# biodatageeks/datafusion-bio-functions

Measured on AMD Instinct MI355X. Metric: overlap-pairs/sec + probe-rows/sec, IntervalJoinExec 100Mx1M, higher is better.
Workload: dtype int32; 1 GPU; join_100Mx1M_24contigs; probe_rows_per_gpu=100000000, build_rows_per_gpu=1000000, contigs=24, pairs_per_gpu=37210484, parallelism=partition-per-gpu x1, gather=False, build_overlap=True

## Files before the change

datafusion-bio-functions_amd/csrc/ivx_capi.hip:

```cpp
#include "ivx_internal.hpp"
#include <cstdlib>
#include <atomic>
#include <chrono>
#include <cstring>
#include <mutex>
#include <new>
#include <thread>
#include <condition_variable>
#include <deque>


void ivx_ctx::join_tail()
{
    if (!tail_pending) return;
    (void)hipStreamWaitEvent(stream, tail_ev, 0);
    tail_pending = false;
}

ivx_status ivx_ctx::get_scratch(int slot, size_t bytes, void **out)
{
    if (tail_pending && slot != WS_SORTHIST && slot != WS_T0 && slot != WS_T1 && slot != WS_T2) join_tail();
    ivx_buf &b = scratch[slot];
    if (sub_plan.valid && ((sub_plan.slots >> slot) & 1)) sub_plan.valid = false;
    if (join_plan.valid && ((join_plan.rows.slots >> slot) & 1)) join_plan.valid = false;
    if (bytes < 256) bytes = 256;
    if (b.cap < bytes) {
        size_t want = bytes + bytes / 8;
        if (mem_limit) {
            const u64 others = reserved() - b.cap;
            if (others + bytes > mem_limit)
                return fail(IVX_ERR_OOM, "Resources exhausted: failed to reserve " + std::to_string(bytes) + " bytes of device scratch (" +
                                         std::to_string(others) + " bytes reserved, limit " + std::to_string(mem_limit) + ")");
            if (others + want > mem_limit) want = bytes;
        }
        if (b.p) { (void)hipStreamSynchronize(stream); if (aux) (void)hipStreamSynchronize(aux); (void)hipFree(b.p); b.p = nullptr; scratch_bytes -= b.cap; b.cap = 0; }
        hipError_t e = hipMalloc(&b.p, want);
        if (e != hipSuccess) { want = bytes; e = hipMalloc(&b.p, want); }
        if (e != hipSuccess) { b.p = nullptr; return fail_hip("hipMalloc(scratch)", e); }
        b.cap = want; scratch_bytes += want;
    }
    *out = b.p;
    return IVX_OK;
}

ivx_status ivx_ctx::get_pinned(int slot, size_t bytes, void **out)
{
    ivx_buf &b = pinned[slot];
    if (bytes < 256) bytes = 256;
    if (b.cap < bytes) {
        if (b.p) { (void)hipStreamSynchronize(stream); (void)hipHostFree(b.p); b.p = nullptr; b.cap = 0; }
        hipError_t e = hipHostMalloc(&b.p, bytes, hipHostMallocDefault);
        if (e != hipSuccess) { b.p = nullptr; return fail_hip("hipHostMalloc", e); }
        b.cap = bytes;
    }
    *out = b.p;
    return IVX_OK;
}

namespace {
struct PoolBuf { void *p; size_t cap; int device; };
std::mutex g_pool_mu;
std::vector<PoolBuf> g_pool;
constexpr size_t POOL_MAX_BUFS = 96;

void *pool_take(int device, size_t bytes, size_t *cap)
{
    std::lock_guard<std::mutex> lk(g_pool_mu);
    size_t best = g_pool.size();
    for (size_t i = 0; i < g_pool.size(); i++) {
        const PoolBuf &b = g_pool[i];
        if (b.device != device || b.cap < bytes || b.cap > 2 * bytes + 4096) continue;
        if (best == g_pool.size() || b.cap < g_pool[best].cap) best = i;
    }
    if (best == g_pool.size()) return nullptr;
    void *p = g_pool[best].p;
    *cap = g_pool[best].cap;
    g_pool.erase(g_pool.begin() + best);
    return p;
}

void pool_give(int device, void *p, size_t cap)
{
    void *drop = nullptr;
    {
        std::lock_guard<std::mutex> lk(g_pool_mu);
        g_pool.push_back({p, cap, device});
        if (g_pool.size() > POOL_MAX_BUFS) { drop = g_pool.front().p; g_pool.erase(g_pool.begin()); }
    }
    if (drop) (void)hipFree(drop);
}

void pool_drop(int device)
{
    std::vector<void *> drop;
    {
        std::lock_guard<std::mutex> lk(g_pool_mu);
        for (size_t i = 0; i < g_pool.size();)
            if (g_pool[i].device == device) { drop.push_back(g_pool[i].p); g_pool.erase(g_pool.begin() + i); }
            else i++;
    }
    for (void *p : drop) (void)hipFree(p);
}
}

ivx_status ivx_index_alloc(ivx_ctx *ctx, ivx_index *ix, size_t bytes, void **out)
{
    if (bytes < 256) bytes = 256;
    if (ctx->mem_limit && ctx->reserved() + bytes > ctx->mem_limit)
        return ctx->fail(IVX_ERR_OOM, "Resources exhausted: failed to reserve " + std::to_string(bytes) + " bytes for the index (" +
// ... 125 lines not shown
    c->stream = c->own_stream;
    if (const char *e = getenv("IVX_BUILD_OVERLAP")) c->overlap = e[0] == '1';
    *out = c;
    return IVX_OK;
}

extern "C" void ivx_ctx_free(ivx_ctx *c)
{
    if (!c) return;
    (void)hipSetDevice(c->device);
    (void)hipStreamSynchronize(c->stream);
    if (c->aux) (void)hipStreamSynchronize(c->aux);
    for (auto &b : c->scratch) if (b.p) (void)hipFree(b.p);
    for (auto &b : c->pinned) if (b.p) (void)hipHostFree(b.p);
    if (c->d_scalars) (void)hipFree(c->d_scalars);
    if (c->h_scalars) (void)hipHostFree(c->h_scalars);
    if (c->ev0) (void)hipEventDestroy(c->ev0);
    if (c->ev1) (void)hipEventDestroy(c->ev1);
    if (c->own_stream) (void)hipStreamDestroy(c->own_stream);
    if (c->aux) (void)hipStreamDestroy(c->aux);
    if (c->ev_fork) (void)hipEventDestroy(c->ev_fork);
    if (c->tail_ev) (void)hipEventDestroy(c->tail_ev);
    delete c;
}

extern "C" const char *ivx_last_error(const ivx_ctx *c) { return c ? c->err.c_str() : "null ctx"; }

extern "C" ivx_status ivx_ctx_set_stream(ivx_ctx *c, void *hip_stream)
{
    if (!c) return IVX_ERR_INVALID;
    if (c->tail_pending) { (void)hipStreamSynchronize(c->aux); c->tail_pending = false; }
    c->stream = (hipStream_t)hip_stream;
    return IVX_OK;
}

extern "C" ivx_status ivx_ctx_use_own_stream(ivx_ctx *c)
{
    if (!c) return IVX_ERR_INVALID;
    if (c->tail_pending) { (void)hipStreamSynchronize(c->aux); c->tail_pending = false; }
    c->stream = c->own_stream;
    return IVX_OK;
}

extern "C" ivx_status ivx_ctx_set_build_overlap(ivx_ctx *c, int on)
{
    if (!c) return IVX_ERR_INVALID;
    c->overlap = on != 0;
    return IVX_OK;
}

extern "C" ivx_status ivx_ctx_synchronize(ivx_ctx *c)
{
    if (!c) return IVX_ERR_INVALID;
    if (c->tail_pending) { IVX_HIP(c, hipStreamSynchronize(c->aux)); c->tail_pending = false; }
    IVX_HIP(c, hipStreamSynchronize(c->stream));
    return IVX_OK;
}

extern "C" ivx_status ivx_ctx_metrics(const ivx_ctx *c, ivx_metrics *out)
{
    if (!c || !out) return IVX_ERR_INVALID;
    *out = c->metrics;
    return IVX_OK;
}

extern "C" void ivx_ctx_reset_metrics(ivx_ctx *c) { if (c) c->metrics = ivx_metrics{}; }

extern "C" ivx_status ivx_ctx_set_memory_limit(ivx_ctx *c, uint64_t bytes)
{
    if (!c) return IVX_ERR_INVALID;
    c->mem_limit = bytes;
    return IVX_OK;
}

extern "C" uint64_t ivx_ctx_reserved_bytes(const ivx_ctx *c) { return c ? c->reserved() : 0; }

extern "C" ivx_status ivx_ctx_trim(ivx_ctx *c, uint64_t keep_bytes)
{
    if (!c) return IVX_ERR_INVALID;
    IVX_HIP(c, hipSetDevice(c->device));
    IVX_HIP(c, hipStreamSynchronize(c->stream));
    if (c->aux) { IVX_HIP(c, hipStreamSynchronize(c->aux)); c->tail_pending = false; }
    c->sub_plan.valid = false; c->join_plan.valid = false;
    while (c->scratch_bytes > keep_bytes) {
        int big = -1;
        for (int i = 0; i < IVX_NSCRATCH; i++)
            if (c->scratch[i].p && (big < 0 || c->scratch[i].cap > c->scratch[big].cap)) big = i;
        if (big < 0) break;
        IVX_HIP(c, hipFree(c->scratch[big].p));
        c->scratch_bytes -= c->scratch[big].cap;
        c->scratch[big] = ivx_buf{};
    }
    pool_drop(c->device);
    return IVX_OK;
}

extern "C" double ivx_ctx_last_kernel_ms(const ivx_ctx *cc)
{
    ivx_ctx *c = const_cast<ivx_ctx *>(cc);
    if (!c) return -1.0;
    if (c->last_ms < 0.0) {
        float ms = 0.f;
        if (hipEventSynchronize(c->ev1) == hipSuccess && hipEventElapsedTime(&ms, c->ev0, c->ev1) == hipSuccess) c->last_ms = ms;
    }
    return c->last_ms;
}


ivx_status ivx_count_build(ivx_ctx *ctx, ivx_index *ix, const u32 *key, const i32 *s, const i32 *e, u64 n);
ivx_status ivx_coverage_build(ivx_ctx *ctx, ivx_index *ix, const u32 *key, const i32 *s, const i32 *e, u64 n);
ivx_status ivx_nearest_build(ivx_ctx *ctx, ivx_index *ix, const u32 *key, const i32 *s, const i32 *e, u64 n);

extern "C" ivx_status ivx_index_build(ivx_ctx *ctx, int kind, int mem, const uint32_t *key, const int32_t *start,
                                      const int32_t *end, uint64_t n, uint32_t n_keys, ivx_index **out)
{
    if (!ctx) return IVX_ERR_INVALID;
    if (!out) return ctx->fail(IVX_ERR_INVALID, "null out");
    *out = nullptr;
    if (kind < IVX_KIND_OVERLAP || kind > IVX_KIND_NEAREST) return ctx->fail(IVX_ERR_INVALID, "bad index kind");
    if (mem != IVX_MEM_HOST && mem != IVX_MEM_DEVICE) return ctx->fail(IVX_ERR_INVALID, "bad mem");
    if (n && (!start || !end)) return ctx->fail(IVX_ERR_INVALID, "null coordinate column");
    if (n > 0xFFFFFFFEull) return ctx->fail(IVX_ERR_INVALID, "build side exceeds UInt32 index capacity");
    if (n_keys == 0) n_keys = 1;
    if (!key) n_keys = 1;
    if (kind == IVX_KIND_NEAREST && n >= 0x80000000ull) return ctx->fail(IVX_ERR_INVALID, "nearest index: more than 2^31-1 rows");
    IVX_HIP(ctx, hipSetDevice(ctx->device));
    ivx_index *ix = new (std::nothrow) ivx_index();
    static std::atomic<u64> next_serial{1};
    if (ix) ix->serial = next_serial.fetch_add(1);
    if (!ix) return ctx->fail(IVX_ERR_OOM, "host allocation failed");
    ix->kind = kind; ix->device = ctx->device; ix->n = n; ix->nkeys = n_keys;
    CallMetrics cm(ctx, true, n);
    ctx->building_bytes = 0;
    const u32 *dk; const i32 *ds, *de;
    ivx_status st = stage_in(ctx, mem, WS_IN_KEY, key, n, &dk);
    if (st == IVX_OK) st = stage_in(ctx, mem, WS_IN_START, start, n, &ds);
    if (st == IVX_OK) st = stage_in(ctx, mem, WS_IN_END, end, n, &de);
    if (st == IVX_OK) {
        KernelTimer t(ctx);
        switch (kind) {
        case IVX_KIND_OVERLAP: st = ivx_join_build(ctx, ix, dk, ds, de, n, mem == IVX_MEM_DEVICE); break;
        case IVX_KIND_COUNT: st = ivx_count_build(ctx, ix, dk, ds, de, n); break;
        case IVX_KIND_COVERAGE: st = ivx_coverage_build(ctx, ix, dk, ds, de, n); break;
        default: st = ivx_nearest_build(ctx, ix, dk, ds, de, n); break;
        }
    }
    if (st == IVX_OK && hipStreamSynchronize(ctx->stream) != hipSuccess) st = ctx->fail(IVX_ERR_HIP, "index build failed on device");
    ctx->building_bytes = 0;
    if (st != IVX_OK) { ivx_index_free(ix); return st; }
    ix->owner_bytes = ctx->live_index_bytes;
    ix->owner_bytes->fetch_add(ix->bytes, std::memory_order_relaxed);
    ctx->metrics.build_mem_used += ix->bytes;
    *out = ix;
    return IVX_OK;
}

extern "C" void ivx_index_free(ivx_index *ix)
{
    if (!ix) return;
    if (ix->ready) { (void)hipEventSynchronize(ix->ready); (void)hipEventDestroy(ix->ready); }
    for (size_t i = 0; i < ix->allocs.size(); i++) pool_give(ix->device, ix->allocs[i], ix->alloc_caps[i]);
    if (ix->owner_bytes) ix->owner_bytes->fetch_sub(ix->bytes, std::memory_order_relaxed);
    delete ix;
}

extern "C" uint64_t ivx_index_rows(const ivx_index *ix) { return ix ? ix->n : 0; }
extern "C" uint64_t ivx_index_device_bytes(const ivx_index *ix) { return ix ? ix->bytes : 0; }

extern "C" ivx_status ivx_index_layout(ivx_ctx *ctx, const ivx_index *ix, uint32_t *out, uint32_t n_out)
{
    if (!ctx) return IVX_ERR_INVALID;
    if (!ix) return ctx->fail(IVX_ERR_INVALID, "null index");
    if (n_out && !out) return ctx->fail(IVX_ERR_INVALID, "null out");
    if (ix->device != ctx->device) return ctx->fail(IVX_ERR_INVALID, "index lives on another device");
    u32 w[IVX_LAYOUT_WORDS] = {};
    w[IVX_LAYOUT_KIND] = (u32)ix->kind;
    if (ix->kind != IVX_KIND_NEAREST && ix->jv.hdr != nullptr) {
        IVX_HIP(ctx, hipSetDevice(ctx->device));
        if (ix->ready != nullptr) IVX_HIP(ctx, hipStreamWaitEvent(ctx->stream, ix->ready, 0));
        u32 h[HDR_WORDS];
        IVX_HIP(ctx, hipMemcpyAsync(h, ix->jv.hdr, sizeof(h), hipMemcpyDeviceToHost, ctx->stream));
        IVX_HIP(ctx, hipStreamSynchronize(ctx->stream));
        const u32 nlev = h[HDR_NLEV] < IVX_MAXL ? h[HDR_NLEV] : IVX_MAXL;
        u32 levrows = 0;
        for (u32 l = 0; l < nlev; l++) if (h[HDR_LEVCNT + l]) levrows |= 1u << l;
        w[IVX_LAYOUT_SH0] = h[HDR_SH0];
        w[IVX_LAYOUT_NLEV] = h[HDR_NLEV];
        w[IVX_LAYOUT_LEVROWS] = levrows;
        w[IVX_LAYOUT_RCELLS] = h[HDR_NREG] ? h[HDR_RCELLS] : 0u;
        w[IVX_LAYOUT_RCS] = h[HDR_NREG] ? h[HDR_CS] : 0xFFFFFFFFu;
        w[IVX_LAYOUT_NREG] = h[HDR_NREG];
        w[IVX_LAYOUT_PK24] = h[HDR_PK24];
        w[IVX_LAYOUT_SLOW] = h[HDR_SLOW];
        w[IVX_LAYOUT_FG] = h[HDR_FG];
        w[IVX_LAYOUT_FBITS] = h[HDR_FG] != 0xFFFFFFFFu ? h[HDR_FBITS] : 0u;
        w[IVX_LAYOUT_NROUTE_NREG] = ix->nroute_nreg;
        w[IVX_LAYOUT_LBUILD] = h[HDR_LBUILD];
    }
    for (u32 i = 0; i < n_out && i < (u32)IVX_LAYOUT_WORDS; i++) out[i] = w[i];
    return IVX_OK;
}


static bool rowval_routed_ok(u64 n)
{
    if (const char *f = getenv("IVX_JOIN_PATH")) return !strcmp(f, "routed");
    return n >= (1u << 21);
}

static ivx_status overlap_common(ivx_ctx *ctx, const ivx_index *ix, int mem, int mode,
                                 const u32 *key, const i32 *start, const i32 *end, u64 n,
                                 u32 *per_row, u8 *exists, u32 *bidx, u32 *pidx, u64 cap, u64 *total)
{
    IVX_TRY(check_probe_args(ctx, ix, IVX_KIND_OVERLAP, mem, start, end, n, true));
    CallMetrics cm(ctx, false, n);
    const u32 *dk = nullptr; const i32 *ds = nullptr, *de = nullptr;
    bool regions = ix->jv_nreg > 0 && (mode == JP_COUNT || mode == JP_FILL) && n >= (1u << 21);
    bool rowval = ix->jv_nreg > 0 && ix->jv_nreg <= IVX_MAXREG_WIDE && (mode == JP_PER_ROW || mode == JP_EXISTS) && n >= (1u << 21);
    if (const char *f = getenv("IVX_JOIN_PATH")) {
        if (!strcmp(f, "direct")) regions = rowval = false;
        else if (!strcmp(f, "regions")) {
            regions = ix->jv_nreg > 0 && (mode == JP_COUNT || mode == JP_FILL);
            rowval = ix->jv_nreg > 0 && ix->jv_nreg <= IVX_MAXREG_WIDE && (mode == JP_PER_ROW || mode == JP_EXISTS);
        }
    }
    const void *in[3] = {key, start, end};
    ivx_join_plan &pl = ctx->join_plan;
    const bool planned = regions && mode == JP_FILL && pl.valid && !getenv("IVX_NO_PLAN") && pl.mem == mem && memcmp(pl.in, in, sizeof(in)) == 0 && pl.n == n &&
                         pl.ix == (const void *)ix && pl.ix_serial == ix->serial && pl.stream == ctx->stream;
    if (ix->ready != nullptr && !(regions && !planned)) IVX_HIP(ctx, hipStreamWaitEvent(ctx->stream, ix->ready, 0));
    if (!planned) {
        IVX_TRY(stage_in(ctx, mem, WS_IN_KEY, key, n, &dk));
        IVX_TRY(stage_in(ctx, mem, WS_IN_START, start, n, &ds));
        IVX_TRY(stage_in(ctx, mem, WS_IN_END, end, n, &de));
    }
    u32 *d_row = nullptr, *d_b = nullptr, *d_p = nullptr; u8 *d_ex = nullptr;
    IVX_TRY(stage_out(ctx, mem, WS_OUT_A, per_row, n, &d_row));
    IVX_TRY(stage_out(ctx, mem, WS_OUT_B, exists, n, &d_ex));
    IVX_TRY(stage_out(ctx, mem, WS_OUT_C, bidx, cap, &d_b));
    IVX_TRY(stage_out(ctx, mem, WS_OUT_D, pidx, cap, &d_p));
    const bool defer_clear = regions && !planned;
    if (!defer_clear) IVX_HIP(ctx, hipMemsetAsync(ctx->d_scalars, 0, 2 * sizeof(u64), ctx->stream));
    {
        KernelTimer t(ctx);
        if (regions) {
            if (!planned) pl.valid = false;
            const ivx_status st = ivx_join_probe_regions(ctx, ix->jv, ix->jv_nreg, mode, dk, ds, de, n, d_b, d_p, cap, ctx->d_scalars, planned, ix->jv_filter, ix->jv_pk24,
                                                         ix->jv_fast_unknown ? 2 : (ix->jv_fast ? 1 : 0), planned ? nullptr : ix->ready, defer_clear);
            if (st != IVX_OK) { pl.valid = false; return st; }
            if (mode == JP_COUNT && pl.valid) { memcpy(pl.in, in, sizeof(in)); pl.mem = mem; pl.n = n; pl.ix = ix; pl.ix_serial = ix->serial; pl.stream = ctx->stream; }
        }
        else if (rowval) IVX_TRY(ivx_rowval_probe_regions(ctx, ix->jv, ix->jv_nreg, mode == JP_PER_ROW ? IVX_RV_PER_ROW : IVX_RV_EXISTS, dk, ds, de, n, 0,
                                                          mode == JP_PER_ROW ? (void *)d_row : (void *)d_ex, ctx->d_scalars, ix->jv_filter, ix->jv_pk24, ix->jv_fast && !ix->jv_fast_unknown));
        else if (n && (mode == JP_PER_ROW || mode == JP_EXISTS) && ix->nroute_nreg > 0 && rowval_routed_ok(n))
            IVX_TRY(ivx_join_rowval_routed(ctx, ix, mode, dk, ds, de, n, d_row, d_ex, ctx->d_scalars));
        else IVX_TRY(ivx_join_probe(ctx, ix->jv, mode, dk, ds, de, n, d_row, d_ex, d_b, d_p, cap, ctx->d_scalars));
    }
    u64 tot = 0;
    if (mode != JP_EXISTS) {
        IVX_HIP(ctx, hipMemcpyAsync(ctx->h_scalars, ctx->d_scalars, 2 * sizeof(u64), hipMemcpyDeviceToHost, ctx->stream));
        IVX_HIP(ctx, hipStreamSynchronize(ctx->stream));
        tot = ctx->h_scalars[0];
        if (ctx->h_scalars[1]) { ctx->join_plan.valid = false; return ctx->fail(IVX_ERR_HIP, "internal error: the probe met an unpublished page of routed rows"); }
    }
    if (mode == JP_COUNT && regions && pl.valid) pl.total = tot;
    if (total) *total = tot;
    if (mode == JP_FILL && tot > cap) return ctx->fail(IVX_ERR_CAPACITY, "pair buffers too small");
    cm.out(mode == JP_FILL ? tot : (mode == JP_COUNT ? 0 : n));
    if (planned) pl.valid = false;
    IVX_TRY(copy_out(ctx, mem, per_row, d_row, n));
    IVX_TRY(copy_out(ctx, mem, exists, d_ex, n));
    if (mode == JP_FILL) { IVX_TRY(copy_out(ctx, mem, bidx, d_b, tot)); IVX_TRY(copy_out(ctx, mem, pidx, d_p, tot)); }
    if (mem == IVX_MEM_HOST) IVX_HIP(ctx, hipStreamSynchronize(ctx->stream));
    return IVX_OK;
}

extern "C" ivx_status ivx_probe_overlap_count(ivx_ctx *ctx, const ivx_index *ix, int mem, const uint32_t *key,
                                              const int32_t *start, const int32_t *end, uint64_t n,
                                              uint32_t *per_row, uint64_t *total)
{
    return overlap_common(ctx, ix, mem, per_row ? JP_PER_ROW : JP_COUNT, key, start, end, n, per_row, nullptr, nullptr, nullptr, 0, total);
}

__global__ void k_add_base(u32 *__restrict__ p, u64 n, u32 base)
{
    for (u64 i = (u64)blockIdx.x * blockDim.x + threadIdx.x; i < n; i += (u64)gridDim.x * blockDim.x) p[i] += base;
}

struct HostCopier {
    struct Job { void *dst; const void *src; size_t bytes; hipEvent_t ev; };
    std::mutex mu; std::condition_variable cv, cv_done; std::deque<Job> jobs; bool closed = false; hipError_t herr = hipSuccess;
    u64 done = 0;
    hipStream_t cs = nullptr; std::thread th; std::vector<hipEvent_t> evs; bool started = false;
    hipError_t start(int device)
    {
        const hipError_t e = hipStreamCreateWithFlags(&cs, hipStreamNonBlocking);
        if (e != hipSuccess) return e;
        try {
        th = std::thread([this, device]() {
            (void)hipSetDevice(device);
            for (;;) {
                Job j;
                { std::unique_lock<std::mutex> lk(mu); cv.wait(lk, [&] { return closed || !jobs.empty(); }); if (jobs.empty()) return; j = jobs.front(); jobs.pop_front(); }
                hipError_t e2 = j.ev ? hipStreamWaitEvent(cs, j.ev, 0) : hipSuccess;
                if (e2 == hipSuccess && j.bytes) e2 = hipMemcpyAsync(j.dst, j.src, j.bytes, hipMemcpyDeviceToHost, cs);
                if (e2 == hipSuccess) e2 = hipStreamSynchronize(cs);
                { std::lock_guard<std::mutex> lk(mu); if (e2 != hipSuccess) herr = e2; done++; }
                cv_done.notify_all();
            }
        });
        } catch (...) { (void)hipStreamDestroy(cs); cs = nullptr; return hipErrorOutOfMemory; }
        started = true;
        return hipSuccess;
    }
    hipError_t mark(hipStream_t st, hipEvent_t *ev)
    {
        hipError_t e = hipEventCreateWithFlags(ev, hipEventDisableTiming);
        if (e != hipSuccess) return e;
        evs.push_back(*ev);
        return hipEventRecord(*ev, st);
    }
    void push(void *dst, const void *src, size_t bytes, hipEvent_t ev)
    {
        { std::lock_guard<std::mutex> lk(mu); jobs.push_back(Job{dst, src, bytes, ev}); }
        cv.notify_all();
    }
    void wait_until(u64 k) { std::unique_lock<std::mutex> lk(mu); cv_done.wait(lk, [&] { return done >= k; }); }
    hipError_t finish()
    {
        if (!started) return hipSuccess;
        { std::lock_guard<std::mutex> lk(mu); closed = true; }
        cv.notify_all();
        th.join();
        for (hipEvent_t e : evs) (void)hipEventDestroy(e);
        (void)hipStreamDestroy(cs);
        started = false;
        return herr;
    }
    ~HostCopier() { (void)finish(); }
};

static ivx_status overlap_fill_host_chunked(ivx_ctx *ctx, const ivx_index *ix, const u32 *key, const i32 *start, const i32 *end, u64 n,
                                            u32 *bidx, u32 *pidx, u64 cap, u64 *written, u32 nchunk)
{
    IVX_TRY(check_probe_args(ctx, ix, IVX_KIND_OVERLAP, IVX_MEM_HOST, start, end, n));
    hipStream_t st = ctx->stream;
// ... 724 lines not shown
```

datafusion-bio-functions_amd/csrc/ivx_internal.hpp:

```cpp
#pragma once
#include <hip/hip_runtime.h>
#include <stdint.h>
#include <atomic>
#include <memory>
#include <string>
#include <vector>
#include "../../include/ivx.h"

typedef uint8_t u8;
typedef uint32_t u32;
typedef int32_t i32;
typedef uint64_t u64;
typedef int64_t i64;

#define IVX_WAVE 64

struct ivx_buf { void *p = nullptr; size_t cap = 0; };

enum { IVX_NSCRATCH = 56, IVX_NPIN = 4 };

struct ivx_sub_plan {
    bool valid = false;
    u64 slots = 0;
    int mem = 0;
    const void *in[6] = {};
    u64 nl = 0, nr = 0, nh = 0, total = 0;
    u32 nkeys = 0;
    int strict = 0;
    hipStream_t stream = nullptr;
    const u32 *lk, *lrow, *rk, *hk, *hj;
    const i64 *lsv, *lev, *rsv, *hrs, *hpm;
    const void *sm;
    const u64 *offs;
    const u32 *plan_hlo; const i64 *plan_tail;
};

struct PageTab { u32 *ptab; u32 pstride, lgpg; };
struct ivx_route_ctl {
    u32 rcur[1024];
    u32 pool_next, pad0[3];
    u32 rest_n[2], pad1[2];
    u32 rfirst[1032];
    u32 cfirst[1032];
};
struct FpRest;
enum {
    IVX_ROWS_FLAT = 0,
    IVX_ROWS_PAGED,
    IVX_ROWS_TABLE
};
struct ivx_routed {
    int form = IVX_ROWS_FLAT;
    const u64 *se = nullptr;
    const u32 *ids = nullptr;
    const unsigned short *cidx = nullptr;
    const u32 *rfirst = nullptr;
    u32 nblk = 1, chunk = 0, ndig = 0;
    const u32 *unsorted = nullptr;
    PageTab pt{nullptr, 0u, 0u};
    bool packed = false;
    u32 rowbits = 32;
    bool all_routed = false;
    ivx_route_ctl *ctl = nullptr;
    FpRest *rest = nullptr; u64 *rest_rows = nullptr;
    const uint2 *vtab = nullptr;
    const i32 *ds = nullptr, *de = nullptr;
    u32 adj = 0;
    u64 slots = 0;
};

struct ivx_join_plan {
    bool valid = false;
    int mem = 0;
    const void *in[3] = {};
    u64 n = 0;
    u64 total = 0;
    const void *ix = nullptr; u64 ix_serial = 0;
    hipStream_t stream = nullptr;
    ivx_routed rows;
};

struct ivx_ctx {
    int device = 0;
    hipStream_t own_stream = nullptr;
    hipStream_t stream = nullptr;
    hipEvent_t ev0 = nullptr, ev1 = nullptr;
    double last_ms = 0.0;
    std::string err;
    ivx_buf scratch[IVX_NSCRATCH];
    ivx_buf pinned[IVX_NPIN];
    u64 *d_scalars = nullptr;
    u64 *h_scalars = nullptr;
    ivx_sub_plan sub_plan;
    ivx_join_plan join_plan;
    ivx_metrics metrics{};
    u64 mem_limit = 0;
    u64 fill_hint = 0;
    u64 scratch_bytes = 0, building_bytes = 0;
    hipStream_t aux = nullptr;
    hipEvent_t ev_fork = nullptr, tail_ev = nullptr;
    bool overlap = false, tail_pending = false;
    void join_tail();
    std::shared_ptr<std::atomic<u64>> live_index_bytes = std::make_shared<std::atomic<u64>>(0);
    u64 reserved() const { return scratch_bytes + building_bytes + live_index_bytes->load(std::memory_order_relaxed); }

    ivx_status fail(ivx_status st, const std::string &msg) { err = msg; return st; }
    ivx_status fail_hip(const char *what, hipError_t e)
    {
        err = std::string(what) + ": " + hipGetErrorString(e);
        return e == hipErrorOutOfMemory ? IVX_ERR_OOM : IVX_ERR_HIP;
    }
    ivx_status get_scratch(int slot, size_t bytes, void **out);
    ivx_status get_pinned(int slot, size_t bytes, void **out);
};

#define IVX_HIP(ctx, call)                                              \
    do {                                                                \
        hipError_t e__ = (call);                                        \
        if (e__ != hipSuccess) return (ctx)->fail_hip(#call, e__);      \
    } while (0)

#define IVX_TRY(call)                                                   \
    do {                                                                \
        ivx_status s__ = (call);                                        \
        if (s__ != IVX_OK) return s__;                                  \
    } while (0)

enum {
    WS_IN_KEY = 0, WS_IN_START, WS_IN_END, WS_IN2_KEY, WS_IN2_START, WS_IN2_END,
    WS_OUT_A, WS_OUT_B, WS_OUT_C, WS_OUT_D, WS_OUT_E, WS_OUT_F, WS_OUT_G, WS_OUT_H,
    WS_SCAN0, WS_SCAN1, WS_SCAN2,
    WS_GRID0, WS_GRID1, WS_GRID2,
    WS_SORTHIST,
    WS_SA0, WS_SA1, WS_SA2, WS_SB0, WS_SB1, WS_SB2,
    WS_RA0, WS_RA1, WS_RA2, WS_RB0, WS_RB1, WS_RB2,
    WS_T0, WS_T1, WS_T2, WS_T3, WS_T4, WS_T5, WS_T6, WS_T7, WS_T8, WS_T9,
    WS_IN3_KEY, WS_IN3_START, WS_IN3_END, WS_IN3_WEIGHT, WS_IN_KEYLEN
};
static_assert(WS_IN_KEYLEN < IVX_NSCRATCH, "scratch slot ids must fit the context's slot array");

#ifndef IVX_LSTEP
#define IVX_LSTEP 2
#endif
#define IVX_MAXL (32 / IVX_LSTEP)
#define IVX_SH_MIN 4

struct ivx_ent { i32 s, e; u32 row; };

enum { HDR_SH0 = 0, HDR_NLEV = 1, HDR_NBINS = 2, HDR_CS = 3 , HDR_NREG = 4,
       HDR_RCELLS = 5 , HDR_RMUL_LO = 6, HDR_RMUL_HI = 7 , HDR_LEVCNT = 8 ,
       HDR_FG = 8 + IVX_MAXL , HDR_FBITS = 9 + IVX_MAXL ,
       HDR_PK24 = 10 + IVX_MAXL ,
       HDR_SLOW = 11 + IVX_MAXL ,
       HDR_LBUILD = 12 + IVX_MAXL ,
       HDR_BADKEY = 13 + IVX_MAXL ,
       HDR_WORDS = 14 + IVX_MAXL };
#define IVX_FBITS_MAX (1u << 24)
#define IVX_MAXREG 255
#define IVX_MAXREG_WIDE 1023
#define IVX_MAXREG2 65025u
#define IVX_REG_CS_MAX 13

#ifndef IVX_RP_ECAP
#define IVX_RP_ECAP 6144
#endif
#define IVX_RP_HALO 8u
struct ivx_regdesc { u32 k; i32 origin; u32 span, lb, slo, shi, e0, ne; i32 rbase;  };

struct JoinIndexView {
    const i32 *origin;
    const u32 *span;
    const u32 *kcnt;
    const u32 *lbase;
    const u32 *binstart;
    const ivx_ent *ent;
    const u32 *hdr;
    const u32 *kreg;
    const u32 *rkey;
    const ivx_regdesc *rdesc;
    const u32 *fbits;
    const u32 *fbase;
    u32 nkeys;
};

struct RankGridView {
    const i32 *origin;
    const u32 *span;
    const u32 *kcnt;
    const u32 *koff;
    const u32 *kbase;
    const u32 *binstart;
    const i32 *val;
    const u32 *hdr;
    u32 nkeys;
};

struct CoverageView {
    RankGridView first, last;
    const i64 *pw;
    const i32 *nfirst, *nlast;
};

struct ivx_nrec { i32 a, b; u32 row; i32 pmax; };

struct NearestView {
    RankGridView by_start, by_end, pmax;
    const ivx_nrec *rs;
    const ivx_nrec *re;
    JoinIndexView ov;
};

struct ivx_index {
    u64 serial = 0;
    int kind = 0;
    int device = 0;
    u64 n = 0;
    u32 nkeys = 0;
    size_t bytes = 0;
    std::shared_ptr<std::atomic<u64>> owner_bytes;
    std::vector<void *> allocs;
    std::vector<size_t> alloc_caps;
    JoinIndexView jv{};
    u32 jv_nreg = 0;
    bool jv_filter = false;
    bool jv_pk24 = false;
    bool jv_fast = false;
    bool jv_fast_unknown = false;
    hipEvent_t ready = nullptr;
    RankGridView gs{}, ge{};
    CoverageView cv{};
    NearestView nv{};
    JoinIndexView nroute{};
    u32 nroute_nreg = 0;
    int flags = 0;
};
enum { IVX_IXF_REGION_ROWVAL = 1 };

ivx_status ivx_scan_exclusive_u32(ivx_ctx *ctx, u32 *data, u64 n, const u32 *skip = nullptr);
ivx_status ivx_scan_exclusive_u64(ivx_ctx *ctx, u64 *data, u64 n);

ivx_status ivx_join_build(ivx_ctx *ctx, ivx_index *ix, const u32 *key, const i32 *s, const i32 *e, u64 n, bool overlap = false);
ivx_status ivx_join_probe(ivx_ctx *ctx, const JoinIndexView &jv, int mode,
                          const u32 *key, const i32 *s, const i32 *e, u64 n,
                          u32 *per_row, u8 *exists, u32 *ob, u32 *op, u64 cap, u64 *d_cursor);
enum { JP_COUNT = 0, JP_PER_ROW = 1, JP_EXISTS = 2, JP_FILL = 3 };
ivx_status ivx_join_probe_regions(ivx_ctx *ctx, const JoinIndexView &jv, u32 nreg, int mode,
                                  const u32 *key, const i32 *s, const i32 *e, u64 n,
                                  u32 *ob, u32 *op, u64 cap, u64 *d_cursor, bool planned = false, bool has_filter = false, bool pk24 = false,
                                  int fast = 0 , hipEvent_t ready = nullptr,
                                  bool clear_cursor = false );

enum { IVX_RV_COUNT = 0, IVX_RV_COVERAGE = 1, IVX_RV_PER_ROW = 2, IVX_RV_EXISTS = 3 };
ivx_status ivx_route_view_build(ivx_ctx *ctx, ivx_index *ix, const i32 *origin, const u32 *span, const u32 *kcnt);
void ivx_route_view_ready(ivx_ctx *ctx, ivx_index *ix);
ivx_status ivx_join_rowval_routed(ivx_ctx *ctx, const ivx_index *ix, int mode, const u32 *key, const i32 *s, const i32 *e, u64 n,
                                  u32 *per_row, u8 *exists, u64 *d_total);
ivx_status ivx_unroute_u32(ivx_ctx *ctx, const ivx_routed &r, u64 n, const u32 *vb, u32 *out32, u8 *out8);
ivx_status ivx_route_rows(ivx_ctx *ctx, const JoinIndexView &rv, const u32 *key, const i32 *s, const i32 *e, u64 n, u32 adj, ivx_routed *out);
ivx_status ivx_unroute_pair(ivx_ctx *ctx, const ivx_routed &r, u64 n, const u32 *vb, const i64 *vd, u32 *ob, u32 *op, i64 *od, i64 dflt);
ivx_status ivx_rowval_probe_regions(ivx_ctx *ctx, const JoinIndexView &jv, u32 nreg, int kind,
                                    const u32 *key, const i32 *s, const i32 *e, u64 n, int strict, void *out, u64 *d_total,
                                    bool has_filter = false, bool pk24 = false, bool fast = false);

ivx_status ivx_mark_probe(ivx_ctx *ctx, const JoinIndexView &jv, const u32 *key, const i32 *s, const i32 *e, u64 n, u32 *marks);
ivx_status ivx_mark_probe_regions(ivx_ctx *ctx, const JoinIndexView &jv, u32 nreg, const u32 *key, const i32 *s, const i32 *e, u64 n,
                                  u32 *marks, bool has_filter, bool pk24, bool fast, bool *took);
ivx_status ivx_bits_mark_device(ivx_ctx *ctx, const u32 *idx, u64 n, u32 *bits, u64 n_bits);
ivx_status ivx_bits_select_device(ivx_ctx *ctx, const u32 *bits, u64 n_bits, int want_set, u32 *out, u64 cap, u64 *n_out);

ivx_status ivx_depth_device(ivx_ctx *ctx, const u32 *rkey, const u32 *rpos, const u32 *rflags, const u32 *rmapq,
                            const i32 *cigar_offsets, const u32 *cigar_ops, u64 n_reads,
                            const u32 *skey, const u32 *sstart, const u32 *send, const i32 *sweight, u64 n_seg,
                            u32 nkeys, const u32 *key_len, u32 filter_flag, u32 min_mapq,
                            u32 *ok, u32 *os, u32 *oe, i32 *oc, u64 cap, u64 *n_out);

ivx_status ivx_index_alloc(ivx_ctx *ctx, ivx_index *ix, size_t bytes, void **out);
```

datafusion-bio-functions_amd/csrc/ivx_join.hip:

```cpp
#include <cstdlib>
#include <cstring>
#include "ivx_device.hpp"
#include "ivx_grid.hpp"
#include "ivx_join.hpp"

namespace {

constexpr int BT = 256;

constexpr int LB_T = 1024;
constexpr int LB_ROWS = 4;
constexpr u32 LB_TILE = LB_T * LB_ROWS;
constexpr u32 LB_STRIDE = IVX_MAXREG_WIDE + 1;
constexpr u32 LB_CCAP = 8192;
constexpr u32 LB_MAXTILES = 1024;
constexpr int LB_KEEP = (IVX_RP_ECAP + LB_T - 1) / LB_T;
constexpr u64 LB_MIN_ROWS = 1u << 14, LB_MAX_ROWS = (u64)LB_MAXTILES * LB_TILE;
static_assert(LB_STRIDE == LB_T && LB_TILE <= 4096 && LB_CCAP == (1u << IVX_REG_CS_MAX), "k_lbuild_tiles: one table word per thread, 12-bit ranks");
static inline u32 lb_tstride(u32 ntiles) { return ntiles | 1u; }


__device__ __forceinline__ u32 cells_of(u32 cnt, u32 span, u32 sh) { return cnt ? (sh >= 32 ? 1u : (span >> sh) + 1u) : 0u; }

__global__ __launch_bounds__(1024) void k_join_layout(const i32 *kmin, const i32 *kmax, const u32 *kcnt, u32 nkeys, u64 n,
// ... 542 lines not shown


ivx_status ivx_route_view_build(ivx_ctx *ctx, ivx_index *ix, const i32 *origin, const u32 *span, const u32 *kcnt)
{
    hipStream_t st = ctx->stream;
    const u32 nkeys = ix->nkeys;
    u32 *kreg, *rkey, *rhdr;
    IVX_TRY(ivx_index_alloc(ctx, ix, ((size_t)nkeys + 1) * sizeof(u32), (void **)&kreg));
    IVX_TRY(ivx_index_alloc(ctx, ix, ((size_t)IVX_MAXREG_WIDE + 1) * sizeof(u32), (void **)&rkey));
    IVX_TRY(ivx_index_alloc(ctx, ix, HDR_WORDS * sizeof(u32), (void **)&rhdr));
    IVX_HIP(ctx, hipMemsetAsync(rhdr, 0, HDR_WORDS * sizeof(u32), st));
    hipLaunchKernelGGL(k_nroute_layout, dim3(1), dim3(1024), 0, st, origin, span, kcnt, nkeys, kreg, rkey, rhdr);
    IVX_HIP(ctx, hipMemcpyAsync(ctx->h_scalars + 48, rhdr, HDR_WORDS * sizeof(u32), hipMemcpyDeviceToHost, st));
    ix->nroute = JoinIndexView{};
    ix->nroute.origin = origin; ix->nroute.span = span; ix->nroute.kcnt = kcnt; ix->nroute.kreg = kreg; ix->nroute.rkey = rkey;
    ix->nroute.hdr = rhdr; ix->nroute.nkeys = nkeys;
    IVX_HIP(ctx, hipGetLastError());
    return IVX_OK;
}
void ivx_route_view_ready(ivx_ctx *ctx, ivx_index *ix) { ix->nroute_nreg = ((const u32 *)(ctx->h_scalars + 48))[HDR_NREG]; }

ivx_status ivx_join_rowval_routed(ivx_ctx *ctx, const ivx_index *ix, int mode, const u32 *key, const i32 *s, const i32 *e, u64 n,
                                  u32 *per_row, u8 *exists, u64 *d_total)
{
    hipStream_t st = ctx->stream;
    ivx_routed R;
    IVX_TRY(ivx_route_rows(ctx, ix->nroute, key, s, e, n, 0u, &R));
    u32 *vb;
    IVX_TRY(ctx->get_scratch(WS_T2, n * sizeof(u32), (void **)&vb));
    const u32 grid = (ivx_stream_grid(n, PT * 4, 1280u) + 7u) & ~7u;
    hipLaunchKernelGGL(k_overlap_rowval_routed, dim3(grid), dim3(PT), 0, st, ix->jv, ix->nroute.rkey, ix->nroute_nreg, R.se, R.rfirst, R.nblk,
                       mode == JP_EXISTS ? 1 : 0, vb, (unsigned long long *)d_total, R.unsorted);
    IVX_TRY(ivx_unroute_u32(ctx, R, n, vb, per_row, exists));
    const u32 g2 = ivx_stream_grid(n, PTILE, 256 * 8);
    if (mode == JP_PER_ROW) hipLaunchKernelGGL((k_probe_overlap<JP_PER_ROW, PI>), dim3(g2), dim3(PT), 0, st, ix->jv, key, s, e, n, per_row, exists, (u32 *)nullptr, (u32 *)nullptr, (u64)0, (unsigned long long *)d_total, R.unsorted);
    else hipLaunchKernelGGL((k_probe_overlap<JP_EXISTS, PI>), dim3(g2), dim3(PT), 0, st, ix->jv, key, s, e, n, per_row, exists, (u32 *)nullptr, (u32 *)nullptr, (u64)0, (unsigned long long *)d_total, R.unsorted);
    IVX_HIP(ctx, hipGetLastError());
    return IVX_OK;
}

ivx_status ivx_join_build(ivx_ctx *ctx, ivx_index *ix, const u32 *key, const i32 *s, const i32 *e, u64 n, bool overlap)
{
    const u32 nkeys = ix->nkeys;
    hipStream_t st = ctx->stream;
    const u64 maxcells = 2 * n + (IVX_LSTEP >= 4 ? n / 4 : n) + (u64)IVX_MAXL * nkeys + 64;
    if (maxcells + 1 >= 0xFFFFFFFFull) return ctx->fail(IVX_ERR_INVALID, "build side too large for 32-bit cell ids");

    i32 *origin; u32 *span, *kcnt, *lbase, *binstart, *hdr, *kreg, *rkey, *fbase, *fbits; ivx_ent *ent; ivx_regdesc *rdesc;
    IVX_TRY(ivx_index_alloc(ctx, ix, nkeys * sizeof(i32), (void **)&origin));
    IVX_TRY(ivx_index_alloc(ctx, ix, nkeys * sizeof(u32), (void **)&span));
    IVX_TRY(ivx_index_alloc(ctx, ix, nkeys * sizeof(u32), (void **)&kcnt));
    IVX_TRY(ivx_index_alloc(ctx, ix, (size_t)IVX_MAXL * nkeys * sizeof(u32), (void **)&lbase));
    IVX_TRY(ivx_index_alloc(ctx, ix, (maxcells + 1) * sizeof(u32), (void **)&binstart));
    IVX_TRY(ivx_index_alloc(ctx, ix, HDR_WORDS * sizeof(u32), (void **)&hdr));
    IVX_TRY(ivx_index_alloc(ctx, ix, ((size_t)nkeys + 1) * sizeof(u32), (void **)&kreg));
    size_t regcap = (size_t)(n / (IVX_RP_ECAP / 2)) + (size_t)(maxcells >> IVX_REG_CS_MAX) + 2 * (size_t)nkeys + 64;
    regcap = regcap <= IVX_MAXREG + 1 ? (size_t)IVX_MAXREG + 1 : (regcap > (size_t)IVX_MAXREG2 + 1 ? (size_t)IVX_MAXREG2 + 1 : regcap);
    IVX_TRY(ivx_index_alloc(ctx, ix, regcap * sizeof(u32), (void **)&rkey));
    IVX_TRY(ivx_index_alloc(ctx, ix, regcap * sizeof(ivx_regdesc), (void **)&rdesc));
    IVX_TRY(ivx_index_alloc(ctx, ix, (n ? n : 1) * sizeof(ivx_ent), (void **)&ent));
    const size_t fwords = IVX_FBITS_MAX / 32 + 4;
    IVX_TRY(ivx_index_alloc(ctx, ix, nkeys * sizeof(u32), (void **)&fbase));
    IVX_TRY(ivx_index_alloc(ctx, ix, fwords * sizeof(u32), (void **)&fbits));

    i32 *kmin, *kmax; u32 *cellid, *rank, *errflag;
    IVX_TRY(ctx->get_scratch(WS_GRID0, nkeys * sizeof(i32), (void **)&kmin));
    IVX_TRY(ctx->get_scratch(WS_GRID1, nkeys * sizeof(i32), (void **)&kmax));
    const char *benv = getenv("IVX_BUILD");
    const bool lb_try = n >= LB_MIN_ROWS && n <= LB_MAX_ROWS && !(benv && !strcmp(benv, "global"));
    const u32 lb_tiles = lb_try ? (u32)((n + LB_TILE - 1) / LB_TILE) : 0u;
    IVX_TRY(ctx->get_scratch(WS_GRID2, (n ? n : 1) * (lb_try ? sizeof(ivx_ent) : sizeof(u32)), (void **)&cellid));
    const size_t tabbytes = (size_t)lb_tstride(lb_tiles) * LB_STRIDE * sizeof(u32);
    IVX_TRY(ctx->get_scratch(WS_T9, (n ? n : 1) * sizeof(u32) > tabbytes ? (n ? n : 1) * sizeof(u32) : tabbytes, (void **)&rank));
    errflag = (u32 *)(ctx->d_scalars + 8);
    u32 *lenhist = (u32 *)(ctx->d_scalars + 32);

    ivx_zero_ranges zr{{errflag, lenhist, hdr}, {1u, 34u, (u32)HDR_WORDS}};
    const char *fenv = getenv("IVX_FILTER");
    const int filter_mode = !fenv ? 1 : !strcmp(fenv, "0") ? 0 : !strcmp(fenv, "force") ? 2 : 1;
    static_assert((IVX_FBITS_MAX / 32 + 4) % 4 == 0, "the bitmap is cleared in 16-byte words");
    if (filter_mode) { zr.big = (uint4 *)fbits; zr.nbig = (u32)(fwords / 4); }
    IVX_TRY(ivx_keystats_len(ctx, key, s, n, nkeys, kmin, kmax, kcnt, errflag, 1u, e, lenhist, &zr));
    const u32 grid = ivx_stream_grid(n, BT * 2, 16384);
    hipLaunchKernelGGL(k_join_layout, dim3(1), dim3(1024), 0, st, kmin, kmax, kcnt, nkeys, n, origin, span, lbase, hdr, maxcells, kreg, rkey, (const u32 *)lenhist, (u32)(regcap - 1), fbase, filter_mode, lb_try ? 1 : 0, (const u32 *)errflag);
    if (filter_mode) hipLaunchKernelGGL(k_join_filter, dim3(grid), dim3(BT), 0, st, key, s, e, n, nkeys, (const i32 *)origin, (const u32 *)span, (const u32 *)fbase, (const u32 *)hdr, fbits);
    const bool want_route = ix->kind == IVX_KIND_OVERLAP && n >= (4u << 20);
    overlap = overlap && ctx->overlap && ctx->aux != nullptr && !want_route && n >= (1u << 16);
    hipStream_t tail_st = st;
    struct TailGuard {
        ivx_ctx *c; bool armed = false;
        ~TailGuard() { if (armed) (void)hipStreamSynchronize(c->aux); }
    } guard{ctx};
    bool q_lds = lb_try, q_global = true;
    if (overlap) {
        ctx->join_tail();
        IVX_HIP(ctx, hipEventRecord(ctx->ev_fork, st));
        IVX_HIP(ctx, hipStreamWaitEvent(ctx->aux, ctx->ev_fork, 0));
        tail_st = ctx->aux;
        IVX_HIP(ctx, hipMemcpyAsync(ctx->h_scalars + 32, hdr, HDR_WORDS * sizeof(u32), hipMemcpyDeviceToHost, st));
        IVX_HIP(ctx, hipStreamSynchronize(st));
        if (((const u32 *)(ctx->h_scalars + 32))[HDR_BADKEY]) return ctx->fail(IVX_ERR_INVALID, "build key id >= n_keys");
        q_lds = lb_try && ((const u32 *)(ctx->h_scalars + 32))[HDR_LBUILD] != 0;
        q_global = !q_lds;
        guard.armed = true;
    }
    if (q_lds)
        hipLaunchKernelGGL(k_lbuild_tiles, dim3(lb_tiles), dim3(LB_T), 0, tail_st, key, s, e, n, nkeys, (const i32 *)origin, (const u32 *)kreg, hdr,
                           (ivx_ent *)cellid, rank, lb_tstride(lb_tiles), binstart, maxcells + 1);
    else
        IVX_HIP(ctx, hipMemsetAsync(binstart, 0, (maxcells + 1) * sizeof(u32), tail_st));
    if (q_global) {
        hipLaunchKernelGGL(k_join_count, dim3(grid), dim3(BT), 0, tail_st, key, s, e, n, nkeys, origin, lbase, hdr, binstart, cellid, rank);
        const hipStream_t keep = ctx->stream;
        ctx->stream = tail_st;
        const ivx_status sst = ivx_scan_exclusive_u32(ctx, binstart, maxcells + 1, hdr + HDR_LBUILD);
        ctx->stream = keep;
        IVX_TRY(sst);
        hipLaunchKernelGGL(k_join_scatter, dim3(grid), dim3(BT), 0, tail_st, s, e, n, (const u32 *)binstart, (const u32 *)cellid, (const u32 *)rank, ent, (const u32 *)hdr);
    }
    if (q_lds) {
        const u32 rgrid = regcap - 1 < IVX_MAXREG_WIDE ? (u32)(regcap - 1) : (u32)IVX_MAXREG_WIDE;
        hipLaunchKernelGGL(k_lbuild_regions, dim3(rgrid), dim3(LB_T), 0, tail_st, (const i32 *)origin, (const u32 *)span, (const u32 *)lbase, (const u32 *)kreg,
                           (const u32 *)rkey, (const u32 *)hdr, nkeys, (const ivx_ent *)cellid, (const u32 *)rank, lb_tiles, lb_tstride(lb_tiles), binstart, ent);
    }
    hipLaunchKernelGGL(k_join_regdesc, dim3((u32)((regcap + 255) / 256)), dim3(256), 0, tail_st, origin, span, lbase, hdr, kreg, rkey, binstart, rdesc);
    IVX_HIP(ctx, hipGetLastError());
    if (overlap) {
        if (ix->ready == nullptr) IVX_HIP(ctx, hipEventCreateWithFlags(&ix->ready, hipEventDisableTiming));
        IVX_HIP(ctx, hipEventRecord(ix->ready, ctx->aux));
        IVX_HIP(ctx, hipEventRecord(ctx->tail_ev, ctx->aux));
        ctx->tail_pending = true;
        ix->jv_fast_unknown = true;
    }
    if (want_route) IVX_TRY(ivx_route_view_build(ctx, ix, origin, span, kcnt));

    if (!overlap) {
        IVX_HIP(ctx, hipMemcpyAsync(ctx->h_scalars + 32, hdr, HDR_WORDS * sizeof(u32), hipMemcpyDeviceToHost, st));
        IVX_HIP(ctx, hipStreamSynchronize(st));
    }
    if (((const u32 *)(ctx->h_scalars + 32))[HDR_BADKEY]) return ctx->fail(IVX_ERR_INVALID, "build key id >= n_keys");
    ix->jv_nreg = ((const u32 *)(ctx->h_scalars + 32))[HDR_NREG];
    ix->jv_filter = ((const u32 *)(ctx->h_scalars + 32))[HDR_FG] != 0xFFFFFFFFu;
    ix->jv_pk24 = ((const u32 *)(ctx->h_scalars + 32))[HDR_PK24] != 0;
    ix->jv_fast = ((const u32 *)(ctx->h_scalars + 32))[HDR_SLOW] == 0 && ix->jv_nreg > 0;
    if (want_route) ivx_route_view_ready(ctx, ix);
    guard.armed = false;

    ix->jv.origin = origin; ix->jv.span = span; ix->jv.kcnt = kcnt; ix->jv.lbase = lbase;
    ix->jv.binstart = binstart; ix->jv.ent = ent; ix->jv.hdr = hdr; ix->jv.nkeys = nkeys;
    ix->jv.kreg = kreg; ix->jv.rkey = rkey; ix->jv.rdesc = rdesc;
    ix->jv.fbits = fbits; ix->jv.fbase = fbase;
    return IVX_OK;
}

ivx_status ivx_join_probe(ivx_ctx *ctx, const JoinIndexView &jv, int mode,
                          const u32 *key, const i32 *s, const i32 *e, u64 n,
                          u32 *per_row, u8 *exists, u32 *ob, u32 *op, u64 cap, u64 *d_cursor)
{
    if (n == 0) return IVX_OK;
    unsigned long long *cur = (unsigned long long *)d_cursor;
    const bool small = n <= (1u << 18);
    const u32 grid = small ? (u32)((n + PT - 1) / PT) : ivx_stream_grid(n, PTILE, 256 * 8);
#define IVX_PROBE_LAUNCH(M_) do { \
        if (small) hipLaunchKernelGGL((k_probe_overlap<M_, 1>), dim3(grid), dim3(PT), 0, ctx->stream, jv, key, s, e, n, per_row, exists, ob, op, cap, cur, (const u32 *)nullptr); \
        else hipLaunchKernelGGL((k_probe_overlap<M_, PI>), dim3(grid), dim3(PT), 0, ctx->stream, jv, key, s, e, n, per_row, exists, ob, op, cap, cur, (const u32 *)nullptr); \
    } while (0)
    switch (mode) {
    case JP_COUNT: IVX_PROBE_LAUNCH(JP_COUNT); break;
    case JP_PER_ROW: IVX_PROBE_LAUNCH(JP_PER_ROW); break;
    case JP_EXISTS: IVX_PROBE_LAUNCH(JP_EXISTS); break;
    default: IVX_PROBE_LAUNCH(JP_FILL); break;
    }
#undef IVX_PROBE_LAUNCH
    IVX_HIP(ctx, hipGetLastError());
    return IVX_OK;
}
```

datafusion-bio-functions_amd/csrc/ivx_join.hpp:

```cpp
#pragma once
#include "ivx_device.hpp"

__device__ __forceinline__ u32 level_of(i32 s, i32 e, u32 sh0, u32 nlev)
{
    i64 len = (i64)e - (i64)s;
    if (len <= 0) return 0;
    u32 bits = 64 - __clzll((u64)len);
    u32 l = bits <= sh0 ? 0 : (bits - sh0 + IVX_LSTEP - 1) / IVX_LSTEP;
    return l < nlev ? l : nlev - 1;
}

__device__ __forceinline__ u32 cell_of(const i32 *origin, const u32 *lbase, u32 nkeys, u32 k, i32 s, u32 l, u32 sh0)
{
    const u32 sh = sh0 + IVX_LSTEP * l;
    const u32 off = (u32)((i64)s - (i64)origin[k]);
    return lbase[(u64)l * nkeys + k] + (sh >= 32 ? 0u : off >> sh);
}

template <class F>
__device__ __forceinline__ void walk_ent(const JoinIndexView &ix, u32 sh0, u32 lev0, u32 nlev, u32 k, i32 qs, i32 qe, F &&f)
{
    if (k >= ix.nkeys) return;
    if (ix.kcnt[k] == 0) return;
    const i32 origin = ix.origin[k];
    const u32 span = ix.span[k];
    const i64 hi64 = (i64)qe - (i64)origin;
    if (hi64 < 0) return;
    for (u32 l = lev0; l < nlev; l++) {
        if (ix.hdr[HDR_LEVCNT + l] == 0) continue;
        const u32 sh = sh0 + IVX_LSTEP * l;
        u32 blo = 0, bhi = 0;
        if (sh < 32) {
            const u32 ncell = (span >> sh) + 1u;
            const i64 lo64 = (i64)qs - ((i64)1 << sh) + 1 - (i64)origin;
            const i64 bl = lo64 <= 0 ? 0 : (lo64 >> sh);
            const i64 bh = hi64 >> sh;
            if (bl >= (i64)ncell) continue;
            blo = (u32)bl;
            bhi = bh >= (i64)ncell ? ncell - 1u : (u32)bh;
            if (blo > bhi) continue;
        }
        const u32 base = ix.lbase[(u64)l * ix.nkeys + k];
        const u32 a = ix.binstart[base + blo], b = ix.binstart[base + bhi + 1];
        for (u32 j = a; j < b; j++) {
            const ivx_ent x = ix.ent[j];
            if (x.s <= qe && x.e >= qs) f(x);
        }
    }
}
template <class F>
__device__ __forceinline__ void walk(const JoinIndexView &ix, u32 sh0, u32 lev0, u32 nlev, u32 k, i32 qs, i32 qe, F &&f)
{
    walk_ent(ix, sh0, lev0, nlev, k, qs, qe, [&](const ivx_ent &x) { f(x.row); });
}

__device__ __forceinline__ void mark_bit(u32 *bits, u32 i)
{
    u32 *w = bits + (i >> 5);
    const u32 b = 1u << (i & 31u);
    if ((*w & b) == 0u) atomicOr(w, b);
}
```

datafusion-bio-functions_amd/csrc/ivx_regions_probe.hip:

```cpp
#include "ivx_regions.hpp"

namespace {


#ifndef IVX_RP_B
#define IVX_RP_B 8
#endif
#ifndef IVX_RP_RING
#define IVX_RP_RING 512
#endif
#ifndef IVX_RP_ECAP
#define IVX_RP_ECAP 6144
#endif
constexpr int RP_B = IVX_RP_B;
constexpr u32 RP_HALO = IVX_RP_HALO;
constexpr u32 RP_CCAP = 8192 + RP_HALO + 2;
constexpr u32 RP_ECAP = IVX_RP_ECAP;
constexpr u32 RP_RING = IVX_RP_RING;
constexpr u32 RP_NSLOT = 4;
constexpr u32 RP_NPG = 64;
constexpr u32 RP_STASH = 48;
constexpr u32 FD_SLOT_SHIFT = 13;
#ifndef IVX_FD_HEAD
#define IVX_FD_HEAD 3
// ... 221 lines not shown
                if (!(qe[q] < qs[q])) walk(q, [&](u32, bool, i32, i32) { v++; });
            } else if (KIND == RV_MATCHES) {
                walk(q, [&](u32, bool, i32, i32) { v++; });
            } else {
                const i32 a = rv_wadd(qe[q], 1), b = rv_wsub(qs[q], 1);
                walk(q, [&](u32, bool, i32 first, i32 last) {
                    const i32 d = rv_wsub(a < last ? a : last, b > first ? b : first);
                    v = (u32)rv_wadd((i32)v, d > 1 ? d : 1);
                });
            }
        }
        val[q] = v;
    }
}

__device__ __forceinline__ void round_publish(const ProbeLds &L, u32 mine, u32 round, u32 wv, unsigned long long *cursor)
{
    if (lane_id() != 0) return;
    const u32 sl = round % RP_NSLOT;
    L.s_wcnt[sl][wv] = mine;
    const u32 before = __hip_atomic_fetch_add(&L.s_arrive[sl], 1u, __ATOMIC_ACQ_REL, __HIP_MEMORY_SCOPE_WORKGROUP);
    if (before != RP_W - 1) return;
    u32 tot = 0;
#pragma unroll
    for (int w = 0; w < RP_W; w++) tot += L.s_wcnt[sl][w];
    L.s_base[sl] = tot ? atomicAdd(cursor, (unsigned long long)tot) : 0ull;
    __hip_atomic_store(&L.s_arrive[sl], 0u, __ATOMIC_RELAXED, __HIP_MEMORY_SCOPE_WORKGROUP);
    __hip_atomic_store(&L.s_ready[sl], round + 1u, __ATOMIC_RELEASE, __HIP_MEMORY_SCOPE_WORKGROUP);
}

__device__ __forceinline__ u64 round_wait(const ProbeLds &L, u32 round, u32 wv, u64 cap, bool &fits)
{
    const u32 sl = round % RP_NSLOT;
    while (__hip_atomic_load(&L.s_ready[sl], __ATOMIC_ACQUIRE, __HIP_MEMORY_SCOPE_WORKGROUP) != round + 1u)
        __builtin_amdgcn_s_sleep(1);
    const u64 base = L.s_base[sl];
    u64 g = base;
    u32 tot = 0;
#pragma unroll
    for (int w = 0; w < RP_W; w++) { const u32 c = L.s_wcnt[sl][w]; if (w < (int)wv) g += c; tot += c; }
    fits = base + tot <= cap;
    return g;
}

__device__ __forceinline__ void round_copy_out(const ProbeLds &L, u32 mine, u32 start, u32 round, u32 wv,
                                               u32 *ob, u32 *op, u64 cap)
{
    bool fits;
    const u64 g = round_wait(L, round, wv, cap, fits);
    if (!mine || !fits) return;
    for (u32 t = lane_id(); t < mine; t += IVX_WAVE) {
        const u64 x = L.s_q[wv][(start + t) & (RP_RING - 1)];
        ob[g + t] = (u32)x; op[g + t] = (u32)(x >> 32);
    }
}

#define IVX_PROBE_LDS(FILL)                                                                          \
    __shared__ unsigned short s_off[RP_CCAP];                                                        \
    __shared__ u64 s_ent[RP_ECAP];                                                                   \
    __shared__ u32 s_row[RP_ECAP];                                                                   \
    __shared__ u64 s_q[FILL ? RP_W : 1][RP_RING];                                                    \
    __shared__ u32 s_wpos[RP_W];                                                                     \
    __shared__ u32 s_wcnt[RP_NSLOT][RP_W];                                                           \
    __shared__ unsigned long long s_base[RP_NSLOT];                                                  \
    __shared__ u32 s_arrive[RP_NSLOT], s_ready[RP_NSLOT];                                            \
    if (threadIdx.x < RP_W) s_wpos[threadIdx.x] = 0;                                                 \
    if (threadIdx.x < RP_NSLOT) { s_arrive[threadIdx.x] = 0; s_ready[threadIdx.x] = 0; }             \
    ProbeLds L{s_off, s_ent, s_row, s_q, s_wpos, s_wcnt, s_base, s_arrive, s_ready};

__global__ void k_pick_rows(const u32 *__restrict__ rfirst, u32 nreg, u64 hint, u32 force, u32 *bsel)
{
    const u32 routed = rfirst[nreg];
    const float per_row = (float)((double)hint / (double)(routed ? routed : 1u));
    *bsel = force ? force : per_row <= 0.40f ? 8u : per_row <= 0.8f ? 4u : per_row <= 1.6f ? 2u : 1u;
}

template <int MODE, int B, bool IDENT, bool PAGED = false, bool PK = false>
__global__ __launch_bounds__(RP_T) void k_probe_regions(JoinIndexView ix, const void *__restrict__ rows_a, const void *__restrict__ rows_b,
                                                        const u32 *__restrict__ offs, u32 nblk, u32 vpb,
                                                        u32 *__restrict__ ob, u32 *__restrict__ op, u64 cap,
                                                        unsigned long long *cursor, u32 prow_stride, u32 adj,
                                                        const u32 *unsorted, PageTab pt = PageTab{nullptr, 0u, 0u},
                                                        const u32 *bsel = nullptr, const i32 *__restrict__ ps_in = nullptr, const i32 *__restrict__ pe_in = nullptr,
                                                        u32 rowbits = 32, const u32 *only_if_set = nullptr)
{
    constexpr bool FILL = MODE == 1;
    if (only_if_set != nullptr && *only_if_set == 0u) return;
    const u32 rowmask = rowbits >= 32 ? 0xFFFFFFFFu : (1u << rowbits) - 1u;
    const u32 maxlen = pk_maxlen(rowbits);
    static_assert(!PK || PAGED, "packed rows come from the one-pass partition");
    if (bsel != nullptr && *bsel != (u32)B) return;
    if ((unsorted != nullptr && *unsorted == 0) != IDENT) return;
    static_assert(!(IDENT && PAGED), "paged rows are never read in place");
    __shared__ u32 s_pg[RP_NPG];
    u32 pg_first = 0;
    auto row_at = [&](u64 i, u32, u64 rf) -> u64 {
        if (!PAGED) return i;
        const u32 x = (u32)(i - rf);
        const u32 pg = s_pg[(x >> pt.lgpg) - pg_first] - 1u;
        return ((u64)pg << pt.lgpg) + (x & ((1u << pt.lgpg) - 1u));
    };
    auto pages_load = [&](u64 lo, u64 &c_hi, u32 r, u64 rf) {
        if (!PAGED) return;
        __syncthreads();
        pg_first = (u32)(lo - rf) >> pt.lgpg;
        const u64 lim = (rf + ((u64)(pg_first + RP_NPG) << pt.lgpg)) & ~63ull;
        if (c_hi > lim) c_hi = lim;
        const u32 npg = ((u32)(c_hi - 1 - rf) >> pt.lgpg) - pg_first + 1u;
        if (threadIdx.x < npg) {
            u32 v = pt.ptab[(u64)r * pt.pstride + pg_first + threadIdx.x];
            if (v == 0u) { v = 1u; if (cursor != nullptr) atomicOr((unsigned int *)(cursor + 1), 1u); }
            s_pg[threadIdx.x] = v;
        }
        __syncthreads();
    };
    auto row_se = [&](u64 i) -> u64 {
        if (IDENT) return (u64)(u32)((u32)((const i32 *)rows_a)[i] + adj) | ((u64)(u32)((u32)((const i32 *)rows_b)[i] - adj) << 32);
        return ((const u64 *)rows_a)[i];
    };
    auto row_id = [&](u64 i, u64 at) -> u32 { return IDENT ? (u32)i : ((const u32 *)rows_b)[at * prow_stride]; };
    constexpr u32 WB = IVX_WAVE * B;
    IVX_PROBE_LDS(FILL)
    const u32 wv = threadIdx.x / IVX_WAVE, ln = lane_id();
    const u32 nreg = ix.hdr[HDR_NREG];
    __shared__ u32 s_rfirst[IVX_MAXREG_WIDE + 2];
    const bool rf_lds = nreg <= IVX_MAXREG_WIDE;
    if (rf_lds) for (u32 t = threadIdx.x; t <= nreg; t += RP_T) s_rfirst[t] = offs[(u64)t * nblk];
    __syncthreads();
    auto rfirst = [&](u32 r) -> u32 { return rf_lds ? s_rfirst[r] : offs[(u64)r * nblk]; };
    const u64 total_rows = rfirst(nreg);
    const u32 nvb = gridDim.x * vpb;
    u32 loaded_r = 0xFFFFFFFFu;
    Slice S;
    slice_init(ix, S, L);
    u32 round = 0;
    u32 pend_mine = 0, pend_start = 0;
    for (u32 vb = blockIdx.x * vpb; vb < (blockIdx.x + 1) * vpb; vb++) {
        u64 lo = total_rows * vb / nvb;
        const u64 hi = total_rows * (vb + 1) / nvb;
        u64 wcur = 0;
        if (lo < hi) {
            u32 r;
            {
                u32 a = 0, b = nreg;
                while (a < b) { const u32 m = (a + b + 1) >> 1; if (rfirst(m) <= lo) a = m; else b = m - 1; }
                r = a;
            }
            for (; lo < hi; r++) {
                const u64 rend = rfirst(r + 1);
                u64 c_hi = hi < rend ? hi : rend;
                if (c_hi <= lo) continue;
                u64 nx[B]; u32 nxr[B];
                u64 b0 = lo + (u64)wv * IVX_WAVE;
                const u64 rf = PAGED ? rfirst(r) : 0;
                pages_load(lo, c_hi, r, rf);
                u64 nat0 = 0, cat0 = 0;
                auto prefetch = [&](u64, u64 bl) -> bool {
                    if (PAGED) {
                        const u64 i0 = bl + ln, i7 = i0 + (u64)(B - 1) * (RP_W * IVX_WAVE);
                        const u32 x0 = (u32)(i0 - rf), x7 = (u32)(i7 - rf);
                        const bool one = i7 < c_hi && (x0 >> pt.lgpg) == (x7 >> pt.lgpg);
                        if (__ballot(!one) == 0) {
                            const u64 at0 = row_at(i0, r, rf);
                            nat0 = at0;
#pragma unroll
                            for (int q = 0; q < B; q++) {
                                const u64 at = at0 + (u64)q * (RP_W * IVX_WAVE);
                                nx[q] = row_se(at);
                                nxr[q] = (FILL && !PK) ? row_id(i0 + (u64)q * (RP_W * IVX_WAVE), at) : 0u;
                            }
// ... 125 lines not shown
    {
        const u32 c = c_lo + i / SUB, sb = i % SUB;
        while (c >= s_cfirst[r + 1]) r++;
        first = (c - s_cfirst[r]) * FP_CHUNK + wv * (8u * IVX_WAVE) + sb * WB;
        const u32 rows = rcur[r];
        cnt = rows > first ? (rows - first < WB ? rows - first : WB) : 0u;
        if (cnt) {
            src = routed_word(pt, pool, r, first, miss);
#pragma unroll
            for (int q = 0; q < B; q++) nx[q] = src[q * IVX_WAVE + ln];
        }
    }
    template <class Miss>
    __device__ __forceinline__ Batch take(u32 i, u32 (&rel)[B], u32 (&len)[B], u32 (&hi)[B], Miss &&miss)
    {
        const Batch b{first, cnt, src};
#pragma unroll
        for (int q = 0; q < B; q++) { const PkRow w = pk_unpack(nx[q], rowbits); rel[q] = w.rel; len[q] = w.len; hi[q] = w.hi; }
        if (i + 1 < nbatch) prefetch(i + 1, miss);
        return b;
    }
};

template <int B, bool FULL>
__device__ __forceinline__ void lean_cells_of(const Slice &S, const u32 (&rel)[B], const u32 (&len)[B], u32 maxlen, u32 cnt, u32 ln,
                                              u32 (&ca)[B], u32 (&cb)[B], u32 &slow, u32 &okm)
{
    const u32 sh0 = S.sh0, off = S.off, cmax = S.cmax, ncm1 = S.ncm1;
#pragma unroll
    for (int q = 0; q < B; q++) {
        const u32 t = ((rel[q] + 1u) >> sh0) + off;
        const u32 bl0 = (t > 1u ? t : 1u) - 1u;
        const u32 bh0 = ((rel[q] + len[q]) >> sh0) + off;
        const u32 bh = bh0 < cmax ? bh0 : cmax;
        bool bad = len[q] == maxlen || bh >= ncm1;
        const bool ok = FULL || (u32)q * IVX_WAVE + ln < cnt;
        if (ok && bad) slow |= 1u << q;
        if (ok && !bad) okm |= 1u << q;
        bad |= !ok;
        const u32 e1 = bad ? 0u : bh + 1u;
        const u32 bl = bl0 < e1 ? bl0 : e1;
        ca[q] = S.s_off[bl];
        cb[q] = S.s_off[e1];
    }
}
template <int B>
__device__ __forceinline__ void lean_cells(const Slice &S, const u32 (&rel)[B], const u32 (&len)[B], u32 maxlen, u32 cnt, u32 ln,
                                           u32 (&ca)[B], u32 (&cb)[B], u32 &slow, u32 &okm)
{
    slow = 0; okm = 0;
    if (cnt == IVX_WAVE * B) lean_cells_of<B, true>(S, rel, len, maxlen, cnt, ln, ca, cb, slow, okm);
    else lean_cells_of<B, false>(S, rel, len, maxlen, cnt, ln, ca, cb, slow, okm);
}

template <int B>
__device__ __forceinline__ void lean_list_slow(u32 slow, u32 r, u32 first, u32 ln, u64 *__restrict__ rest_rows, u32 *rest_n)
{
#pragma unroll
    for (int q = 0; q < B; q++)
        if ((slow >> q) & 1u) rest_rows[atomicAdd(rest_n + 1, 1u)] = (u64)(first + (u32)q * IVX_WAVE + ln) | ((u64)r << 32);
}

template <class W> struct RestRow { W *slot; u32 row, hi; i32 qs, qe; };
template <class W, class Miss>
__device__ __forceinline__ RestRow<W> rest_row(const JoinIndexView &ix, const PageTab &pt, W *pool, u32 r, u32 v, u32 rowbits,
                                               const i32 *ps_in, const i32 *pe_in, u32 adj, Miss &&miss)
{
    W *slot = routed_word(pt, pool, r, v, miss);
    const PkRow w = pk_unpack(*slot, rowbits);
    const u32 row = w.hi & (rowbits >= 32 ? 0xFFFFFFFFu : (1u << rowbits) - 1u);
    i32 qs, qe;
    if (w.len == pk_maxlen(rowbits)) { qs = (i32)((u32)ps_in[row] + adj); qe = (i32)((u32)pe_in[row] - adj); }
    else { qs = (i32)((u32)ix.rdesc[r].rbase + w.rel); qe = (i32)((u32)qs + w.len); }
    return RestRow<W>{slot, row, w.hi, qs, qe};
}

template <int B, bool DRAIN>
__global__ __launch_bounds__(RP_T) void k_fill_fast(JoinIndexView ix, const u64 *__restrict__ pool, const u32 *__restrict__ rcur,
                                                    const u32 *__restrict__ cfirst, PageTab pt, u32 *__restrict__ ob, u32 *__restrict__ op, u64 cap,
                                                    unsigned long long *cursor, const u32 *bsel, u32 rowbits, FpRest *__restrict__ rest, u64 *__restrict__ rest_rows, u32 *rest_n,
                                                    u32 drain)
{
    if (bsel != nullptr && *bsel != (u32)B) return;
    if (ix.hdr[HDR_SLOW] != 0u) return;
    IVX_PROBE_LDS(true)
    __shared__ u32 s_cfirst[IVX_MAXREG_WIDE + 2];
    __shared__ u32 s_wat[RP_NSLOT][RP_W];
    __shared__ u32 s_stash[DRAIN ? RP_W : 1][RP_STASH];
    const u32 wv = __builtin_amdgcn_readfirstlane(threadIdx.x / IVX_WAVE), ln = lane_id();
    auto miss = [&]() { if (ln == 0) atomicOr((unsigned int *)(cursor + 1), 1u); };
    LeanRows<B, const u64> rows;
    if (!rows.init(ix, s_cfirst, cfirst, rcur, pt, pool, rowbits)) return;
    Slice S;
    slice_init(ix, S, L);
    rows.start(miss);
    const u32 rowmask = rowbits >= 32 ? 0xFFFFFFFFu : (1u << rowbits) - 1u;
    u32 loaded_r = 0xFFFFFFFFu;
    u32 round = 0;
    u32 pend_mine = 0;
    constexpr u32 HALF = RP_RING / 2;
    auto copy_out = [&](u32 pr) {
        const u32 sl = pr % RP_NSLOT;
        while (__hip_atomic_load(&L.s_ready[sl], __ATOMIC_ACQUIRE, __HIP_MEMORY_SCOPE_WORKGROUP) != pr + 1u) __builtin_amdgcn_s_sleep(1);
        if (!pend_mine) return;
        const u64 base = L.s_base[sl];
        const u32 tot = s_wat[sl][RP_W - 1] + L.s_wcnt[sl][RP_W - 1];
        if (base + tot > cap) return;
        const u64 g = base + s_wat[sl][wv];
        u32 *ob_w = ob + g, *op_w = op + g;
        const uint2 *half = (const uint2 *)L.s_q[wv] + (pr & 1u) * HALF;
        for (u32 t = ln; t < pend_mine; t += IVX_WAVE) {
            const uint2 x = half[t];
            ob_w[t] = L.s_row[x.x]; op_w[t] = x.y & rowmask;
        }
    };
    for (u32 i = 0; i < rows.nbatch; i++) {
        const u32 r = rows.r;
        if (r != loaded_r) {
            if (round) { copy_out(round - 1u); pend_mine = 0; }
            slice_load(ix, S, L, r, true);
            loaded_r = r;
        }
        u32 rel[B], len[B], roww[B];
        const auto bt = rows.take(i, rel, len, roww, miss);
        const u32 first = bt.first, cnt = bt.cnt;
        const i32 rbase = S.rbase;
        u32 ca[B], cb[B], slow, okm;
        lean_cells<B>(S, rel, len, rows.maxlen, cnt, ln, ca, cb, slow, okm);
        u32 wpos = 0;
        uint2 *half = (uint2 *)L.s_q[wv] + (round & 1u) * HALF;
        auto step = [&](u32 &j, u32 jend, i32 qs, i32 qe, u32 rw, u64 &actm) {
            const u64 x = L.s_ent[j];
            const u64 mm = actm & __builtin_amdgcn_sicmp((i32)(u32)x, qe, 41 ) & __builtin_amdgcn_sicmp((i32)(u32)(x >> 32), qs, 39 );
            if (__builtin_amdgcn_inverse_ballot_w64(mm)) half[mask_rank_from(mm, wpos) & (HALF - 1)] = make_uint2(j, rw);
            wpos += (u32)__popcll(mm);
            j++;
            actm = __builtin_amdgcn_uicmp(j, jend, 36 );
        };
        u32 sfill = 0;
#pragma unroll
        for (int q = 0; q < B; q++) {
            const i32 qs = (i32)((u32)rbase + rel[q]), qe = (i32)((u32)qs + len[q]);
            u32 j = ca[q];
            const u32 jend = cb[q];
            u64 actm = __builtin_amdgcn_uicmp(j, jend, 36);
            if constexpr (!DRAIN) {
                if (actm != 0) {
                    do step(j, jend, qs, qe, roww[q], actm); while (actm != 0);
                }
            } else {
                const u32 lim = drain < RP_STASH - sfill ? drain : RP_STASH - sfill;
                if ((u32)__popcll(actm) > lim) {
#pragma unroll
                    for (int h = 0; h < FD_HEAD; h++) step(j, jend, qs, qe, roww[q], actm);
                    while ((u32)__popcll(actm) > lim) step(j, jend, qs, qe, roww[q], actm);
                }
                if (actm != 0) {
                    if (__builtin_amdgcn_inverse_ballot_w64(actm)) s_stash[wv][mask_rank_from(actm, sfill)] = j | (((u32)q * IVX_WAVE + ln) << FD_SLOT_SHIFT);
                    sfill += (u32)__popcll(actm);
                }
            }
        }
        if (DRAIN && sfill != 0) {
            __builtin_amdgcn_fence(__ATOMIC_RELEASE, "wavefront");
            __builtin_amdgcn_wave_barrier();
            __builtin_amdgcn_fence(__ATOMIC_ACQUIRE, "wavefront");
            const bool has = ln < sfill;
            const u32 e = has ? s_stash[wv][ln] : 0u;
            const PkRow w = pk_unpack(bt.src[e >> FD_SLOT_SHIFT], rowbits);
            const i32 qs = (i32)((u32)rbase + w.rel), qe = (i32)((u32)qs + w.len);
            const u32 bh0 = ((w.rel + w.len) >> S.sh0) + S.off;
            u32 j = e & ((1u << FD_SLOT_SHIFT) - 1u);
            const u32 jend = has ? (u32)S.s_off[(bh0 < S.cmax ? bh0 : S.cmax) + 1u] : 0u;
            u64 actm = __builtin_amdgcn_uicmp(j, jend, 36);
            while (actm != 0) step(j, jend, qs, qe, w.hi, actm);
        }
        u32 got = wpos;
        const bool skip = got > HALF;
        if (__builtin_expect(skip, 0)) {
            if (ln < B && ln * IVX_WAVE < cnt) rest[atomicAdd(rest_n, 1u)] = FpRest{r, first + ln * IVX_WAVE, cnt - ln * IVX_WAVE < IVX_WAVE ? cnt - ln * IVX_WAVE : (u32)IVX_WAVE, 0u};
            got = 0;
        } else if (__builtin_expect(slow != 0, 0)) lean_list_slow<B>(slow, r, first, ln, rest_rows, rest_n);
        if (ln == 0) {
            const u32 sl = round % RP_NSLOT;
            L.s_wcnt[sl][wv] = got;
            const u32 before = __hip_atomic_fetch_add(&L.s_arrive[sl], 1u, __ATOMIC_ACQ_REL, __HIP_MEMORY_SCOPE_WORKGROUP);
            if (before == RP_W - 1) {
                u32 tot = 0;
#pragma unroll
                for (int w = 0; w < RP_W; w++) { s_wat[sl][w] = tot; tot += L.s_wcnt[sl][w]; }
                L.s_base[sl] = tot ? atomicAdd(cursor, (unsigned long long)tot) : 0ull;
                __hip_atomic_store(&L.s_arrive[sl], 0u, __ATOMIC_RELAXED, __HIP_MEMORY_SCOPE_WORKGROUP);
                __hip_atomic_store(&L.s_ready[sl], round + 1u, __ATOMIC_RELEASE, __HIP_MEMORY_SCOPE_WORKGROUP);
            }
        }
        if (round) copy_out(round - 1u);
        pend_mine = got; round++;
    }
    if (round) copy_out(round - 1u);
}

__global__ __launch_bounds__(256) void k_fill_rest(JoinIndexView ix, const u64 *__restrict__ pool, PageTab pt, const FpRest *__restrict__ rest,
                                                   const u64 *__restrict__ rest_rows, const u32 *__restrict__ rest_n, u32 *__restrict__ ob,
                                                   u32 *__restrict__ op, u64 cap, unsigned long long *cursor, const i32 *__restrict__ ps_in,
                                                   const i32 *__restrict__ pe_in, u32 rowbits)
{
    const u32 nbat = rest_n[0], nrow = rest_n[1];
    if (nbat == 0 && nrow == 0) return;
    const u32 wpb = blockDim.x / IVX_WAVE, ln = lane_id();
    const u32 sh0 = ix.hdr[HDR_SH0], nlev = ix.hdr[HDR_NLEV];
    auto rows64 = [&](bool ok, u32 r, u32 v) {
        i32 qs = 0, qe = -1; u32 row = 0, k = 0;
        if (ok) {
            const auto e = rest_row(ix, pt, pool, r, v, rowbits, ps_in, pe_in, 0u, [&]() { atomicOr((unsigned int *)(cursor + 1), 1u); });
            qs = e.qs; qe = e.qe; row = e.row;
            k = ix.rkey[r];
        }
        u32 m = 0;
        if (ok) walk(ix, sh0, 0, nlev, k, qs, qe, [&](u32) { m++; });
        const u32 inc = wave_incl_scan(m);
        const u32 tot = __shfl(inc, IVX_WAVE - 1, IVX_WAVE);
        if (tot == 0) return;
        unsigned long long g = 0;
        if (ln == 0) g = atomicAdd(cursor, (unsigned long long)tot);
        g = __shfl(g, 0, IVX_WAVE);
        if (g + tot > cap) return;
        u64 at = g + inc - m;
        if (m) walk(ix, sh0, 0, nlev, k, qs, qe, [&](u32 brow) { ob[at] = brow; op[at] = row; at++; });
    };
    const u32 wave = blockIdx.x * wpb + threadIdx.x / IVX_WAVE, nwave = gridDim.x * wpb;
    for (u32 i0 = wave * IVX_WAVE; i0 < nrow; i0 += nwave * IVX_WAVE) {
        const bool ok = i0 + ln < nrow;
        const u64 e = ok ? rest_rows[i0 + ln] : 0ull;
        rows64(ok, (u32)(e >> 32), (u32)e);
    }
    for (u32 b = wave; b < nbat; b += nwave) {
        const FpRest w = rest[b];
        for (u32 t0 = 0; t0 < w.cnt; t0 += IVX_WAVE) rows64(t0 + ln < w.cnt, w.r, w.first + t0 + ln);
    }
}

#ifndef IVX_RV_WPS
#define IVX_RV_WPS 4
#endif
#ifndef IVX_RV_B
#define IVX_RV_B 8
#endif
template <int KIND, int B>
__global__ __launch_bounds__(RP_T, IVX_RV_WPS) void k_rv_fast(JoinIndexView ix, u64 *__restrict__ pool, const u32 *__restrict__ rcur, const u32 *__restrict__ cfirst,
                                                  PageTab pt, u32 rowbits, u64 *__restrict__ rest_rows, u32 *rest_n)
{
    __shared__ unsigned short s_off[RP_CCAP];
    __shared__ u64 s_ent[RP_ECAP];
    __shared__ u32 s_cfirst[IVX_MAXREG_WIDE + 2];
    ProbeLds L{s_off, s_ent, nullptr, nullptr, nullptr, nullptr, nullptr, nullptr, nullptr};
    const u32 ln = lane_id();
    auto miss = []() {};
    LeanRows<B, u64> rows;
    if (!rows.init(ix, s_cfirst, cfirst, rcur, pt, pool, rowbits)) return;
    Slice S;
    slice_init(ix, S, L);
    rows.start(miss);
    u32 loaded_r = 0xFFFFFFFFu;
    for (u32 i = 0; i < rows.nbatch; i++) {
        const u32 r = rows.r;
        if (r != loaded_r) { slice_load(ix, S, L, r, true); loaded_r = r; }
        u32 rel[B], len[B], roww[B];
        const auto bt = rows.take(i, rel, len, roww, miss);
        u64 *dst = bt.src;
        const i32 rbase = S.rbase;
        u32 ca[B], cb[B], slow, okm;
        lean_cells<B>(S, rel, len, rows.maxlen, bt.cnt, ln, ca, cb, slow, okm);
#pragma unroll
        for (int q = 0; q < B; q++) {
            const i32 qs = (i32)((u32)rbase + rel[q]), qe = (i32)((u32)qs + len[q]);
            const i32 ca1 = rv_wadd(qe, 1), cb1 = rv_wsub(qs, 1);
            u32 v = 0;
            for (u32 j = ca[q]; j < cb[q]; j++) {
                const u64 x = s_ent[j];
                const i32 xs = (i32)(u32)x, xe = (i32)(u32)(x >> 32);
                if (xs <= qe && xe >= qs) {
                    if (KIND == RV_COVERAGE) { const i32 d = rv_wsub(ca1 < xe ? ca1 : xe, cb1 > xs ? cb1 : xs); v = (u32)rv_wadd((i32)v, d > 1 ? d : 1); }
                    else v++;
                }
            }
            if ((okm >> q) & 1u) dst[q * IVX_WAVE + ln] = (u64)v | ((u64)roww[q] << 32);
        }
        if (__builtin_expect(slow != 0, 0)) lean_list_slow<B>(slow, r, bt.first, ln, rest_rows, rest_n);
    }
}

template <int KIND>
__global__ __launch_bounds__(256) void k_rv_rest(JoinIndexView ix, u64 *__restrict__ pool, PageTab pt, const u64 *__restrict__ rest_rows,
                                                 const u32 *__restrict__ rest_n, const i32 *__restrict__ ps_in, const i32 *__restrict__ pe_in,
                                                 u32 rowbits, u32 adj)
{
    const u32 nrow = rest_n[1];
    const u32 sh0 = ix.hdr[HDR_SH0], nlev = ix.hdr[HDR_NLEV];
    for (u32 i = blockIdx.x * blockDim.x + threadIdx.x; i < nrow; i += gridDim.x * blockDim.x) {
        const u64 ent = rest_rows[i];
        const u32 r = (u32)(ent >> 32);
        const auto e = rest_row(ix, pt, pool, r, (u32)ent, rowbits, ps_in, pe_in, adj, []() {});
        const i32 qs = e.qs, qe = e.qe;
        u32 v = 0;
        if (KIND == RV_COVERAGE) {
            const i32 a = rv_wadd(qe, 1), b = rv_wsub(qs, 1);
            walk_ent(ix, sh0, 0, nlev, ix.rkey[r], qs, qe, [&](const ivx_ent &n) {
                const i32 d = rv_wsub(a < n.e ? a : n.e, b > n.s ? b : n.s);
                v = (u32)rv_wadd((i32)v, d > 1 ? d : 1);
            });
        } else if (KIND != RV_COUNT || !(qe < qs)) {
            walk_ent(ix, sh0, 0, nlev, ix.rkey[r], qs, qe, [&](const ivx_ent &) { v++; });
        }
        *e.slot = (u64)v | ((u64)e.hi << 32);
    }
}

template <int B>
__global__ __launch_bounds__(RP_T, IVX_RV_WPS) void k_mark_fast(JoinIndexView ix, const u64 *__restrict__ pool, const u32 *__restrict__ rcur, const u32 *__restrict__ cfirst,
                                                    PageTab pt, u32 rowbits, u64 *__restrict__ rest_rows, u32 *rest_n, u32 *marks)
{
    constexpr u32 NBW = RP_ECAP / 32u;
// ... 199 lines not shown
                            lds = S.inlds && blo >= S.slo && bhi < S.shi;
                            if (lds) { ja = S.s_off[blo - S.slo]; jb = S.s_off[bhi + 1 - S.slo]; }
                            else { ja = ix.binstart[S.lb + blo]; jb = ix.binstart[S.lb + bhi + 1]; }
                        }
                    }
                }
                const u32 la = lds ? ja : 0u, lb = lds ? jb : 0u, ga = lds ? 0u : ja, gb = lds ? 0u : jb;
                walk(la, lb, true);
                if (__any(ga < gb)) walk(ga, gb, false);
            }
            if (S.upper) {
                for (u32 l = 1; l < S.nlev; l++) {
                    if (ix.hdr[HDR_LEVCNT + l] == 0) continue;
                    const u32 sh = S.sh0 + IVX_LSTEP * l;
                    u32 ja = 0, jb = 0;
                    if (live) {
                        u32 blo = 0, bhi = 0; bool any = true;
                        if (sh < 32) {
                            const u32 ncell = (S.span >> sh) + 1u;
                            const i64 lo64 = (i64)qs - ((i64)1 << sh) + 1 - (i64)S.origin;
                            const i64 bl = lo64 <= 0 ? 0 : (lo64 >> sh);
                            const i64 bh = hi64 >> sh;
                            if (bl >= (i64)ncell) any = false;
                            else { blo = (u32)bl; bhi = bh >= (i64)ncell ? ncell - 1u : (u32)bh; if (blo > bhi) any = false; }
                        }
                        if (any) { const u32 lbase = ix.lbase[(u64)l * ix.nkeys + S.k]; ja = ix.binstart[lbase + blo]; jb = ix.binstart[lbase + bhi + 1]; }
                    }
                    if (__any(ja < jb)) walk(ja, jb, false);
                }
            }
        }
        lo = c_hi;
        if (PAGED && lo < hi && lo < rend) r--;
    }
}

struct RegionKnobs {
    bool two_pass;
    bool pack_off;
    bool lean_off;
    bool filter_off;
    const char *dense;
    const char *rp_rows;
    const char *fill_drain;
};
RegionKnobs region_knobs()
{
    auto is = [](const char *name, const char *v) { const char *x = getenv(name); return x && !strcmp(x, v); };
    return RegionKnobs{is("IVX_PART", "two"), is("IVX_PACK", "0"), is("IVX_FILL", "old"), is("IVX_FILTER", "0"), getenv("IVX_DENSE"), getenv("IVX_RP_ROWS"), getenv("IVX_FILL_DRAIN")};
}

int fill_rows_per_lane(const RegionKnobs &K, u64 cap, u64 n)
{
    if (K.rp_rows) return atoi(K.rp_rows);
    const double per_row = (double)cap / (double)n;
    return per_row <= 0.40 ? 8 : per_row <= 0.8 ? 4 : per_row <= 1.6 ? 2 : 1;
}

u32 fill_drain_of(const RegionKnobs &K, int b)
{
    if (K.fill_drain) { const int t = atoi(K.fill_drain); return t <= 0 ? 0u : (u32)t < RP_STASH ? (u32)t : RP_STASH; }
    return b == 8 ? 12u : b == 4 ? 16u : 0u;
}

bool dense_fill_wanted(const RegionKnobs &K, u64 cap, u64 n)
{
    if (K.dense) return atoi(K.dense) != 0;
    return (double)cap / (double)n > 3.5;
}

bool lean_rows_ok(const ivx_routed &R)
{
    return R.form == IVX_ROWS_PAGED && R.packed && R.pt.lgpg >= 13 && R.rest_rows != nullptr;
}

template <int V> using int_tag = std::integral_constant<int, V>;
template <class F> void with_rows_per_lane(int b, F &&f)
{
    switch (b) { case 1: f(int_tag<1>{}); break; case 2: f(int_tag<2>{}); break; case 4: f(int_tag<4>{}); break; default: f(int_tag<8>{}); }
}

template <int MODE, int B>
void launch_probe_regions(hipStream_t st, const JoinIndexView &jv, const ivx_routed &R, u32 grid, u32 *ob, u32 *op, u64 cap,
                          unsigned long long *cur, const u32 *bsel = nullptr, const u32 *only_if_set = nullptr)
{
    const u32 vpb = RP_VGRID / grid;
    if (R.form == IVX_ROWS_PAGED) {
        auto go = [&](auto pk) {
            hipLaunchKernelGGL((k_probe_regions<MODE, B, false, true, IVX_B(pk)>), dim3(grid), dim3(RP_T), 0, st, jv, (const void *)R.se, (const void *)R.ids, R.rfirst, 1u, vpb,
                               ob, op, cap, cur, 1u, R.adj, (const u32 *)nullptr, R.pt, bsel, R.ds, R.de, R.rowbits, only_if_set);
        };
        if constexpr (MODE >= RV_COUNT) go(std::true_type{}); else with_bools(go, R.packed);
        return;
    }
    hipLaunchKernelGGL((k_probe_regions<MODE, B, false>), dim3(grid), dim3(RP_T), 0, st, jv, (const void *)R.se, (const void *)R.ids, R.rfirst, R.nblk, vpb, ob, op, cap, cur, 1u, R.adj, R.unsorted);
    hipLaunchKernelGGL((k_probe_regions<MODE, B, true>), dim3(grid), dim3(RP_T), 0, st, jv, (const void *)R.ds, (const void *)R.de, R.rfirst, R.nblk, vpb, ob, op, cap, cur, 1u, R.adj, R.unsorted);
}

ivx_status dense_fill(ivx_ctx *ctx, const JoinIndexView &jv, u32 nreg, const ivx_routed &R, u64 n, u32 *ob, u32 *op, u64 cap, u64 *d_cursor)
{
    hipStream_t st = ctx->stream;
    const u64 slots = (n >> 6) + nreg + 3;
    u64 *pcount;
    IVX_TRY(ctx->get_scratch(WS_T3, slots * sizeof(u64), (void **)&pcount));
    IVX_HIP(ctx, hipMemsetAsync(pcount, 0, slots * sizeof(u64), st));
    auto pass = [&](auto pass_tag) {
        constexpr int P = decltype(pass_tag)::value;
        if (R.form == IVX_ROWS_PAGED) {
            with_bools([&](auto pk) {
                hipLaunchKernelGGL((k_probe_dense<P, false, true, IVX_B(pk)>), dim3(RP_VGRID), dim3(RP_T), 0, st, jv, (const void *)R.se, (const void *)R.ids, R.rfirst, 1u, 1u,
                                   (const u32 *)nullptr, pcount, ob, op, cap, R.pt, R.ds, R.de, R.rowbits);
            }, R.packed);
            return;
        }
        hipLaunchKernelGGL((k_probe_dense<P, false>), dim3(RP_VGRID), dim3(RP_T), 0, st, jv, (const void *)R.se, (const void *)R.ids, R.rfirst, R.nblk, 1u, R.unsorted, pcount, ob, op, cap);
        hipLaunchKernelGGL((k_probe_dense<P, true>), dim3(RP_VGRID), dim3(RP_T), 0, st, jv, (const void *)R.ds, (const void *)R.de, R.rfirst, R.nblk, 1u, R.unsorted, pcount, ob, op, cap);
    };
    pass(int_tag<0>{});
    IVX_TRY(ivx_scan_exclusive_u64(ctx, pcount, slots));
    IVX_HIP(ctx, hipMemcpyAsync(d_cursor, pcount + (slots - 1), sizeof(u64), hipMemcpyDeviceToDevice, st));
    pass(int_tag<1>{});
    IVX_HIP(ctx, hipGetLastError());
    return IVX_OK;
}

ivx_status probe_pairs(ivx_ctx *ctx, const JoinIndexView &jv, u32 nreg, int mode, const ivx_routed &R, u64 n, u32 *ob, u32 *op, u64 cap,
                       u64 *d_cursor, u64 hint, int fast, bool reused, const RegionKnobs &K)
{
    hipStream_t st = ctx->stream;
    unsigned long long *cur = (unsigned long long *)d_cursor;
    if (mode != JP_FILL) {
        launch_probe_regions<0, RP_B>(st, jv, R, RP_VGRID, ob, op, cap, cur);
        IVX_HIP(ctx, hipGetLastError());
        return IVX_OK;
    }
    if (dense_fill_wanted(K, hint, n)) return dense_fill(ctx, jv, nreg, R, n, ob, op, cap, d_cursor);
    const bool paged = R.form == IVX_ROWS_PAGED;
    u32 *bsel = paged && !R.all_routed ? (u32 *)(ctx->d_scalars + 11) : nullptr;
    if (bsel) hipLaunchKernelGGL(k_pick_rows, dim3(1), dim3(1), 0, st, R.rfirst, nreg, hint, K.rp_rows ? (u32)atoi(K.rp_rows) : 0u, bsel);
    auto every_b = [&](auto &&f) {
        if (bsel) { f(int_tag<8>{}); f(int_tag<4>{}); f(int_tag<2>{}); f(int_tag<1>{}); }
        else with_rows_per_lane(fill_rows_per_lane(K, hint, n), f);
    };
    const u32 *slow_gate = nullptr;
    if (lean_rows_ok(R) && fast != 0 && !K.lean_off && R.rest != nullptr) {
        u32 *rest_n = R.ctl->rest_n;
        if (reused) IVX_HIP(ctx, hipMemsetAsync(rest_n, 0, 2 * sizeof(u32), st));
        every_b([&](auto b) {
            const u32 drain = fill_drain_of(K, decltype(b)::value);
            with_bools([&](auto dr) {
                hipLaunchKernelGGL((k_fill_fast<decltype(b)::value, IVX_B(dr)>), dim3(RP_GRID), dim3(RP_T), 0, st, jv, R.se, (const u32 *)R.ctl->rcur, (const u32 *)R.ctl->cfirst, R.pt, ob, op, cap, cur,
                                   (const u32 *)bsel, R.rowbits, R.rest, R.rest_rows, rest_n, drain);
            }, drain != 0);
        });
        hipLaunchKernelGGL(k_fill_rest, dim3(512), dim3(256), 0, st, jv, R.se, R.pt, (const FpRest *)R.rest, (const u64 *)R.rest_rows, (const u32 *)rest_n, ob, op, cap, cur, R.ds, R.de, R.rowbits);
        IVX_HIP(ctx, hipGetLastError());
        if (fast == 1) return IVX_OK;
        slow_gate = jv.hdr + HDR_SLOW;
    }
    every_b([&](auto b) { launch_probe_regions<1, decltype(b)::value>(st, jv, R, RP_GRID, ob, op, cap, cur, bsel, slow_gate); });
    IVX_HIP(ctx, hipGetLastError());
    return IVX_OK;
}

}

ivx_status ivx_join_probe_regions(ivx_ctx *ctx, const JoinIndexView &jv, u32 nreg, int mode,
                                  const u32 *key, const i32 *s, const i32 *e, u64 n,
                                  u32 *ob, u32 *op, u64 cap, u64 *d_cursor, bool planned, bool has_filter, bool pk24, int fast, hipEvent_t ready, bool clear_cursor)
{
    auto wait_ready = [&]() -> ivx_status { if (ready) { IVX_HIP(ctx, hipStreamWaitEvent(ctx->stream, ready, 0)); ready = nullptr; } return IVX_OK; };
    const RegionKnobs K = region_knobs();
    const bool paged_route = !planned && n != 0 && nreg <= IVX_MAXREG_WIDE && !K.two_pass;
    if (clear_cursor && !paged_route) IVX_HIP(ctx, hipMemsetAsync(d_cursor, 0, 2 * sizeof(u64), ctx->stream));
    if (n == 0) return wait_ready();
    ivx_join_plan &pl = ctx->join_plan;
    ivx_routed R;
    if (planned) R = pl.rows;
    else {
        if (nreg > IVX_MAXREG_WIDE) {
            IVX_TRY(wait_ready());
            IVX_TRY(ivx_route_two_level(ctx, jv, nreg, key, s, e, n, &R));
        } else if (K.two_pass) {
            IVX_TRY(wait_ready());
            IVX_TRY(ivx_route_flat(ctx, jv, key, s, e, n, 0u, nreg > IVX_MAXREG ? 1024u : 256u, false, 4, &R));
        } else {
            IVX_TRY(ivx_route_paged(ctx, jv, nreg, key, s, e, n, ivx_paged_opts{has_filter && !K.filter_off, pk24 && !K.pack_off, false, fast != 0, 0u, clear_cursor ? d_cursor : nullptr}, &R));
        }
        if (mode == JP_COUNT) { pl.rows = R; pl.valid = true; }
    }
    IVX_TRY(wait_ready());
    const u64 hint = ctx->fill_hint ? ctx->fill_hint : (planned && pl.total < cap ? pl.total : cap);
    return probe_pairs(ctx, jv, nreg, mode, R, n, ob, op, cap, d_cursor, hint, fast, planned, K);
}

ivx_status ivx_rowval_probe_regions(ivx_ctx *ctx, const JoinIndexView &jv, u32 nreg, int kind,
                                    const u32 *key, const i32 *s, const i32 *e, u64 n, int strict, void *out, u64 *d_total,
                                    bool has_filter, bool pk24, bool fast)
{
    if (n == 0) return IVX_OK;
    if (nreg == 0 || nreg > IVX_MAXREG_WIDE) return ctx->fail(IVX_ERR_INVALID, "per-row region probe: one partition pass only");
    hipStream_t st = ctx->stream;
    const RegionKnobs K = region_knobs();
    const u32 adj = strict ? 1u : 0u;
    const bool paged = pk24 && nreg <= IVX_MAXREG && !K.two_pass && !K.pack_off;
    ivx_routed R;
    u32 *val = nullptr;
    if (paged) IVX_TRY(ivx_route_paged(ctx, jv, nreg, key, s, e, n, ivx_paged_opts{has_filter && !K.filter_off, true, true, fast && !K.lean_off, adj}, &R));
    else {
        IVX_TRY(ivx_route_flat(ctx, jv, key, s, e, n, adj, nreg > IVX_MAXREG ? 1024u : 256u, true, 2, &R));
        IVX_TRY(ctx->get_scratch(WS_T2, n * sizeof(u32), (void **)&val));
    }
    u64 *pool = const_cast<u64 *>(R.se);
    auto probe = [&](auto kind_tag) {
        constexpr int M = decltype(kind_tag)::value;
        if (lean_rows_ok(R)) {
            hipLaunchKernelGGL((k_rv_fast<M, IVX_RV_B>), dim3(RP_GRID * (IVX_RV_WPS / 4)), dim3(RP_T), 0, st, jv, pool, (const u32 *)R.ctl->rcur, (const u32 *)R.ctl->cfirst, R.pt, R.rowbits, R.rest_rows, R.ctl->rest_n);
            hipLaunchKernelGGL((k_rv_rest<M>), dim3(256), dim3(256), 0, st, jv, pool, R.pt, (const u64 *)R.rest_rows, (const u32 *)R.ctl->rest_n, s, e, R.rowbits, adj);
        } else launch_probe_regions<M, RP_B>(st, jv, R, RP_VGRID, paged ? (u32 *)pool : val, nullptr, 0, nullptr);
    };
    if (kind == IVX_RV_COVERAGE) probe(int_tag<RV_COVERAGE>{}); else if (kind == IVX_RV_COUNT) probe(int_tag<RV_COUNT>{}); else probe(int_tag<RV_MATCHES>{});
    IVX_HIP(ctx, hipGetLastError());
    return ivx_unroute_values(ctx, R, nreg, kind, val, n, out, d_total);
}

ivx_status ivx_mark_probe_regions(ivx_ctx *ctx, const JoinIndexView &jv, u32 nreg, const u32 *key, const i32 *s, const i32 *e, u64 n,
                                  u32 *marks, bool has_filter, bool pk24, bool fast, bool *took)
{
    *took = false;
    const RegionKnobs K = region_knobs();
    if (n == 0 || nreg == 0 || nreg > IVX_MAXREG || !pk24 || !fast || K.two_pass || K.pack_off || K.lean_off) return IVX_OK;
    hipStream_t st = ctx->stream;
    ivx_routed R;
    IVX_TRY(ivx_route_paged(ctx, jv, nreg, key, s, e, n, ivx_paged_opts{has_filter && !K.filter_off, true, true, true, 0u}, &R));
    if (!lean_rows_ok(R)) return IVX_OK;
    hipLaunchKernelGGL((k_mark_fast<IVX_RV_B>), dim3(RP_GRID * (IVX_RV_WPS / 4)), dim3(RP_T), 0, st, jv, R.se, (const u32 *)R.ctl->rcur, (const u32 *)R.ctl->cfirst, R.pt, R.rowbits,
                       R.rest_rows, R.ctl->rest_n, marks);
    hipLaunchKernelGGL(k_mark_rest, dim3(256), dim3(256), 0, st, jv, R.se, R.pt, (const u64 *)R.rest_rows, (const u32 *)R.ctl->rest_n, s, e, R.rowbits, marks);
    IVX_HIP(ctx, hipGetLastError());
    *took = true;
    return IVX_OK;
}
```

datafusion-bio-functions_amd/csrc/ivx_regions_route.hip:

```cpp
#include "ivx_regions.hpp"

namespace {


constexpr int PA_T = 1024;
#ifndef IVX_PA_I
#define IVX_PA_I 12
#endif
constexpr int PA_I = IVX_PA_I;
constexpr int PA_TILE = PA_T * PA_I;
constexpr u32 NO_REGION = 0xFFFFFFFFu;
constexpr u32 KT_MAX = 256;

struct KeyTab {
    bool lds;
    u32 nkeys, sh0, cs;
    u64 rmul;
};

__device__ __forceinline__ void keytab_load(const JoinIndexView &ix, i32 *s_origin, u32 *s_last, u32 *s_kreg, KeyTab &kt)
{
    kt.nkeys = ix.nkeys; kt.sh0 = ix.hdr[HDR_SH0]; kt.cs = ix.hdr[HDR_CS];
    kt.rmul = (u64)ix.hdr[HDR_RMUL_LO] | ((u64)ix.hdr[HDR_RMUL_HI] << 32);
    kt.lds = ix.nkeys <= KT_MAX;
// ... 230 lines not shown
            s_fbase[k] = kt.fg != 0xFFFFFFFFu ? ix.fbase[k] : 0u;
        }
    }
    kt.s_origin = s_origin; kt.s_span = s_span; kt.s_kreg = s_kreg; kt.s_fbase = s_fbase;
}

constexpr u64 PK_ESCAPE = ~0ull;
template <bool KLDS, bool FILT, bool PK>
__device__ __forceinline__ u32 route_prep(const JoinIndexView &ix, const KeyTab2 &kt, u32 k, i32 qs, i32 qe, u32 &fpos, u64 &packed, u32 maxlen)
{
    const bool kok = k < kt.nkeys;
    const u32 kk = kok ? k : 0u;
    const u32 kreg = KLDS ? kt.s_kreg[kk] : (ix.kcnt[kk] ? ix.kreg[kk] : 0xFFFFFFFFu);
    const i32 o = KLDS ? kt.s_origin[kk] : ix.origin[kk];
    const u32 span = KLDS ? kt.s_span[kk] : ix.span[kk];
    const bool hi_ok = qe >= o;
    const bool d_ok = qs >= o;
    const u32 hi32 = (u32)qe - (u32)o, d32 = (u32)qs - (u32)o;
    const bool ok = kok & (kreg != 0xFFFFFFFFu) & hi_ok;
    fpos = 0;
    if (FILT) {
        const u32 lastb = (span >> kt.fg) + 1u;
        const u32 x0 = d_ok ? d32 >> kt.fg : 0u, x1 = hi_ok ? hi32 >> kt.fg : 0u;
        const u32 c0 = x0 > lastb ? lastb : x0, c1 = x1 > lastb ? lastb : x1;
        const u32 b0 = c0 < c1 ? c0 : c1, b1 = c0 < c1 ? c1 : c0;
        const u32 nb1 = b1 - b0;
        const u32 fb = KLDS ? kt.s_fbase[kk] : ix.fbase[kk];
        fpos = ok ? (fb + b0) | ((nb1 > 31u ? 0x3Fu : nb1) << 26) : 0u;
    }
    const u32 last = span >> kt.sh0;
    const u32 cc = d_ok ? d32 >> kt.sh0 : 0u;
    const u32 c = cc > last ? last : cc;
    const u32 rin = kt.cs != 0xFFFFFFFFu ? c >> kt.cs : (u32)(((u64)c * kt.rmul) >> 40);
    packed = PK_ESCAPE;
    if (PK) {
        const u32 rel = d32 - ((rin * kt.rcells) << kt.sh0);
        const u32 len = (u32)qe - (u32)qs;
        if (d_ok && rel < (1u << 24) && qe >= qs && len < maxlen) packed = (u64)rel | ((u64)len << 24);
    }
    return ok ? kreg + rin : NO_REGION;
}

__device__ __forceinline__ bool route_test(u32 fpos, u64 win)
{
    const u32 nb1 = fpos >> 26;
    const u64 m = (2ull << (nb1 & 31u)) - 1ull;
    return (nb1 == 0x3Fu) | (((win >> (fpos & 31u)) & m) != 0);
}


__device__ __forceinline__ u32 page_wait(u32 *slot)
{
    u32 v;
    while ((v = __hip_atomic_load(slot, __ATOMIC_RELAXED, __HIP_MEMORY_SCOPE_AGENT)) == 0u) __builtin_amdgcn_s_sleep(2);
    return v - 1u;
}

template <bool VEC>
__device__ __forceinline__ void load4nt(const u32 *__restrict__ pkey, const i32 *__restrict__ ps, const i32 *__restrict__ pe,
                                        u64 i, u64 hi, u32 (&k)[4], i32 (&s)[4], i32 (&e)[4])
{
    if (VEC && i + 4 <= hi) {
        typedef u32 __attribute__((ext_vector_type(4))) v4u;
        typedef i32 __attribute__((ext_vector_type(4))) v4i;
        const v4u kv = pkey ? __builtin_nontemporal_load(reinterpret_cast<const v4u *>(pkey + i)) : v4u{0u, 0u, 0u, 0u};
        const v4i sv = __builtin_nontemporal_load(reinterpret_cast<const v4i *>(ps + i));
        const v4i ev = __builtin_nontemporal_load(reinterpret_cast<const v4i *>(pe + i));
        k[0] = kv.x; k[1] = kv.y; k[2] = kv.z; k[3] = kv.w;
        s[0] = sv.x; s[1] = sv.y; s[2] = sv.z; s[3] = sv.w;
        e[0] = ev.x; e[1] = ev.y; e[2] = ev.z; e[3] = ev.w;
    } else {
#pragma unroll
        for (int j = 0; j < 4; j++) {
            const bool ok = i + j < hi;
            k[j] = ok ? (pkey ? pkey[i + j] : 0u) : 0xFFFFFFFFu;
            s[j] = ok ? ps[i + j] : 0;
            e[j] = ok ? pe[i + j] : 0;
        }
    }
}

template <bool VEC, int ND, int I, bool KLDS, bool FILT, bool PK, int T = PA_T>
__global__ __launch_bounds__(T, 4) void k_part_onepass(JoinIndexView ix, const u32 *__restrict__ pkey, const i32 *__restrict__ ps,
                                                       const i32 *__restrict__ pe, u64 n, u32 chunk, u32 *__restrict__ rcur, PageTab pt,
                                                       u32 *pool_next, u64 *__restrict__ out_se, u32 *__restrict__ out_row, u32 rowbits,
                                                       u32 adj = 0, uint2 *__restrict__ vtab = nullptr)
{
    constexpr int TILE = T * I;
    static_assert(ND <= T, "one thread per region");
    __shared__ u64 r_se[TILE];
    __shared__ unsigned short r_slot[PK ? 1 : TILE];
    using DigT = typename std::conditional<(ND > 256), unsigned short, unsigned char>::type;
    __shared__ DigT r_dig[TILE];
    __shared__ u32 dstart[ND];
    __shared__ uint2 wtab[ND];
    __shared__ u32 scan_lds[T / IVX_WAVE + 1];
    __shared__ i32 s_origin[KT_MAX];
    __shared__ u32 s_span[KT_MAX], s_kreg[KT_MAX], s_fbase[KT_MAX];

    const u32 tid = threadIdx.x;
    KeyTab2 kt;
    keytab2_load<KLDS>(ix, s_origin, s_span, s_kreg, s_fbase, kt, FILT);
    const u32 pmask = (1u << pt.lgpg) - 1u;
    const u64 lo = (u64)blockIdx.x * chunk;
    const u64 hi = lo + chunk < n ? lo + chunk : n;
    for (u64 t0 = lo; t0 < hi; t0 += TILE) {
        if (tid < ND) dstart[tid] = 0;
        __syncthreads();
        u64 se[PK ? 1 : I]; u32 plo[PK ? I : 1], dig[I];
        constexpr int CH = (I % 8 == 0 && I > 8) ? 8 : I;
#pragma unroll
        for (int c0 = 0; c0 < I; c0 += CH) {
            u32 kk[CH]; i32 qs[CH], qe[CH];
            if (VEC && t0 + TILE <= hi) {
                typedef u32 __attribute__((ext_vector_type(4))) v4u;
                typedef i32 __attribute__((ext_vector_type(4))) v4i;
#pragma unroll
                for (int v = 0; v < CH / 4; v++) {
                    const u64 i = t0 + ((u64)(c0 / 4 + v) * T + tid) * 4;
                    const v4u kv = pkey ? __builtin_nontemporal_load(reinterpret_cast<const v4u *>(pkey + i)) : v4u{0u, 0u, 0u, 0u};
                    const v4i sv = __builtin_nontemporal_load(reinterpret_cast<const v4i *>(ps + i));
                    const v4i ev = __builtin_nontemporal_load(reinterpret_cast<const v4i *>(pe + i));
                    kk[v * 4] = kv.x; kk[v * 4 + 1] = kv.y; kk[v * 4 + 2] = kv.z; kk[v * 4 + 3] = kv.w;
                    qs[v * 4] = sv.x; qs[v * 4 + 1] = sv.y; qs[v * 4 + 2] = sv.z; qs[v * 4 + 3] = sv.w;
                    qe[v * 4] = ev.x; qe[v * 4 + 1] = ev.y; qe[v * 4 + 2] = ev.z; qe[v * 4 + 3] = ev.w;
                }
            } else {
#pragma unroll
                for (int v = 0; v < CH / 4; v++) {
                    u32 k4[4]; i32 s4[4], e4[4];
                    load4nt<false>(pkey, ps, pe, t0 + ((u64)(c0 / 4 + v) * T + tid) * 4, hi, k4, s4, e4);
#pragma unroll
                    for (int j = 0; j < 4; j++) { kk[v * 4 + j] = k4[j]; qs[v * 4 + j] = s4[j]; qe[v * 4 + j] = e4[j]; }
                }
            }
            u32 fpos[CH];
#pragma unroll
            for (int k = 0; k < CH; k++) {
                u64 packed;
                const u32 maxlen = pk_maxlen(rowbits);
                qs[k] = (i32)((u32)qs[k] + adj); qe[k] = (i32)((u32)qe[k] - adj);
                dig[c0 + k] = route_prep<KLDS, FILT, PK>(ix, kt, kk[k], qs[k], qe[k], fpos[k], packed, maxlen);
                if (PK) {
                    const u32 lenf = packed == PK_ESCAPE ? maxlen : (u32)(packed >> 24);
                    plo[PK ? c0 + k : 0] = (packed == PK_ESCAPE ? 0u : (u32)packed & 0xFFFFFFu) | (lenf << 24);
                    fpos[k] = FILT ? fpos[k] : (lenf >> 8);
                } else se[PK ? 0 : c0 + k] = (u64)(u32)qs[k] | ((u64)(u32)qe[k] << 32);
            }
            if (FILT) {
                u64 win[CH];
#pragma unroll
                for (int k = 0; k < CH; k++) __builtin_memcpy(&win[k], kt.fbits + ((fpos[k] & 0x3FFFFFFu) >> 5), sizeof(u64));
#pragma unroll
                for (int k = 0; k < CH; k++) dig[c0 + k] = route_test(fpos[k], win[k]) ? dig[c0 + k] : NO_REGION;
            }
#pragma unroll
            for (int v = 0; v < CH / 4; v++) {
                const u32 d4[4] = {dig[c0 + v * 4], dig[c0 + v * 4 + 1], dig[c0 + v * 4 + 2], dig[c0 + v * 4 + 3]};
                u32 lr[4];
                lds_count_up4(dstart, d4, lr);
#pragma unroll
                for (int u = 0; u < 4; u++) {
                    const int k = v * 4 + u;
                    const u32 lhi = (PK && !FILT) ? fpos[k] << 24 : 0u;
                    dig[c0 + k] = dig[c0 + k] == NO_REGION ? NO_REGION : (dig[c0 + k] | (lr[u] << 10) | lhi);
                }
            }
            if (CH != I) asm volatile("" ::: "memory");
        }
        __syncthreads();
        const u32 mine = tid < ND ? dstart[tid] : 0u;
        u32 v = 0;
        if (mine) v = atomicAdd(&rcur[tid], mine);
        if (vtab && tid < ND) vtab[(u64)(t0 / TILE) * ND + tid] = make_uint2(v, mine);
        u32 tot;
        const u32 ds = block_excl_scan<u32, T>(mine, scan_lds, &tot);
        if (tid < ND) dstart[tid] = ds;
        __syncthreads();
#pragma unroll
        for (int k = 0; k < I; k++) {
            if (dig[k] != NO_REGION) {
                const u32 d = dig[k] & 1023u;
                const u32 pos = dstart[d] + ((dig[k] >> 10) & 0x3FFFu);
                if (PK) {
                    const u32 row = (u32)(t0 + (u32)(((k / 4) * T + tid) * 4 + (k % 4)));
                    r_se[pos] = (u64)plo[PK ? k : 0] | ((u64)(row | (rowbits < 32 ? (dig[k] >> 24) << rowbits : 0u)) << 32);
                } else {
                    r_se[pos] = se[PK ? 0 : k];
                    r_slot[pos] = (unsigned short)(((k / 4) * T + tid) * 4 + (k % 4));
                }
                r_dig[pos] = (DigT)d;
            }
        }
        if (mine) {
            u32 *row = pt.ptab + (u64)tid * pt.pstride;
            const u32 p0 = v >> pt.lgpg, p1 = (v + mine - 1u) >> pt.lgpg;
            const bool own0 = (v & pmask) == 0u, own1 = p1 != p0;
            u32 got = 0;
            if (own0 || own1) {
                got = atomicAdd(pool_next, (own0 ? 1u : 0u) + (own1 ? 1u : 0u));
                if (own0) __hip_atomic_store(&row[p0], got + 1u, __ATOMIC_RELAXED, __HIP_MEMORY_SCOPE_AGENT);
                if (own1) __hip_atomic_store(&row[p1], got + (own0 ? 2u : 1u), __ATOMIC_RELAXED, __HIP_MEMORY_SCOPE_AGENT);
            }
            wtab[tid] = make_uint2(v - ds, (own0 ? got : page_wait(&row[p0])) | (p0 << 16));
        }
        __syncthreads();
#pragma unroll
        for (int k = 0; k < I; k++) {
            const u32 j = k * T + tid;
            if (j < tot) {
                const u32 d = r_dig[j];
                const uint2 w = wtab[d];
                const u32 x = w.x + j;
                u32 pg = w.y & 0xFFFFu;
                if ((x >> pt.lgpg) != (w.y >> 16)) pg = page_wait(pt.ptab + (u64)d * pt.pstride + (x >> pt.lgpg));
                const u64 g = ((u64)pg << pt.lgpg) + (x & pmask);
                out_se[g] = r_se[j];
                if (!PK) out_row[g] = (u32)(t0 + r_slot[j]);
            }
        }
        __syncthreads();
    }
}

__global__ __launch_bounds__(1024) void k_page_bounds(const u32 *__restrict__ rcur, u32 nreg, u32 *__restrict__ rfirst)
{
    __shared__ u32 red[1024 / IVX_WAVE + 1];
    const u32 t = threadIdx.x;
    u32 tot;
    const u32 ex = block_excl_scan<u32, 1024>(t < nreg ? rcur[t] : 0u, red, &tot);
    if (t < nreg) rfirst[t] = ex;
    if (t == 0) rfirst[nreg] = tot;
}

__global__ __launch_bounds__(1024) void k_chunk_bounds(const u32 *__restrict__ rcur, u32 nreg, u32 *__restrict__ rfirst, u32 *__restrict__ cfirst)
{
    __shared__ u32 red[1024 / IVX_WAVE + 1];
    const u32 t = threadIdx.x;
    const u32 rows = t < nreg ? rcur[t] : 0u;
    u32 tot;
    const u32 ex = block_excl_scan<u32, 1024>(rows, red, &tot);
    if (t < nreg) rfirst[t] = ex;
    if (t == 0) rfirst[nreg] = tot;
    __syncthreads();
    const u32 ec = block_excl_scan<u32, 1024>((rows + FP_CHUNK - 1) / FP_CHUNK, red, &tot);
    if (t < nreg) cfirst[t] = ec;
    if (t == 0) cfirst[nreg] = tot;
}

__global__ __launch_bounds__(256) void k_route_clear(u32 *__restrict__ ctl, u32 nctl, u32 *__restrict__ ptab, u64 nptab, u64 *zero2)
{
    const u64 i = (u64)blockIdx.x * 256 + threadIdx.x, step = (u64)gridDim.x * 256;
    if (i < nctl) ctl[i] = 0;
    if (i < 2 && zero2) zero2[i] = 0;
    uint4 *p4 = (uint4 *)ptab;
    for (u64 j = i; j < nptab / 4; j += step) p4[j] = make_uint4(0u, 0u, 0u, 0u);
    if (i < (nptab & 3)) ptab[(nptab & ~3ull) + i] = 0;
}

static inline u32 part_chunk(u64 n, u32 max_tiles = 4) { const u32 t = n >= (16u << 20) ? 4u : n >= (4u << 20) ? 2u : 1u; return (u32)PA_TILE * (t < max_tiles ? t : max_tiles); }

constexpr u32 UP_CHUNK = 2u * PA_TILE;

enum { UP_I64 = 0, UP_I64S = 1, UP_U32 = 2, UP_U8 = 3 };
template <int OUT>
__device__ __forceinline__ void up_store(void *out, u64 i, u32 v)
{
    if (OUT == UP_I64) ((i64 *)out)[i] = (i64)v;
    else if (OUT == UP_I64S) ((i64 *)out)[i] = (i64)(i32)v;
    else if (OUT == UP_U32) ((u32 *)out)[i] = v;
    else ((u8 *)out)[i] = v != 0;
}

template <int OUT, int ND>
__global__ __launch_bounds__(PA_T) void k_unpermute(const u32 *__restrict__ val, const unsigned short *__restrict__ cidx,
                                                    const u32 *__restrict__ offs, u32 nblk, u32 chunk, u32 nreg, u64 n, void *__restrict__ out,
                                                    const u32 *unsorted, unsigned long long *total, int sorted_done = 0)
{
    __shared__ u64 s_sum[PA_T / IVX_WAVE];
    u64 mysum = 0;
    if (*unsorted == 0 && sorted_done) return;
    if (*unsorted == 0) {
        const u64 lo0 = (u64)blockIdx.x * chunk;
        const u64 hi0 = lo0 + chunk < n ? lo0 + chunk : n;
        for (u64 t = lo0 + threadIdx.x; t < hi0; t += PA_T) { const u32 v = val[t]; up_store<OUT>(out, t, v); mysum += v; }
        if (OUT == UP_U32 && total) { const u64 b = block_sum<u64, PA_T>(mysum, s_sum); if (threadIdx.x == 0 && b) atomicAdd(total, (unsigned long long)b); }
        return;
    }
    __shared__ u32 s_val[UP_CHUNK];
    __shared__ u32 s_pre[ND + 1], s_g[ND];
    __shared__ u32 scan_lds[PA_T / IVX_WAVE + 1];
    const u32 tid = threadIdx.x, blk = blockIdx.x;
    const u64 lo = (u64)blk * chunk;
    const u32 len = (u32)(lo + chunk < n ? chunk : n - lo);
    u32 c = 0, g = 0;
    if (tid < nreg) { g = offs[(u64)tid * nblk + blk]; c = offs[(u64)tid * nblk + blk + 1] - g; }
    u32 tot;
    const u32 ex = block_excl_scan<u32, PA_T>(c, scan_lds, &tot);
    if (tid < ND) { s_pre[tid] = ex; s_g[tid] = g; }
    if (tid == 0) s_pre[ND] = tot;
    for (u32 t = tid; t < chunk; t += PA_T) s_val[t] = 0;
    __syncthreads();
    const u32 wv = tid / IVX_WAVE, ln = lane_id();
    const u32 per = (tot + PA_T / IVX_WAVE - 1) / (PA_T / IVX_WAVE);
    const u32 t_lo = wv * per, t_hi = t_lo + per < tot ? t_lo + per : tot;
    u32 r = 0;
    if (t_lo < t_hi) { u32 a = 0, b = ND; while (a < b) { const u32 m = (a + b + 1) >> 1; if (s_pre[m] <= t_lo + ln && m < ND) a = m; else b = m - 1; } r = a; }
    for (u32 t = t_lo + ln; t < t_hi; t += IVX_WAVE) {
        while (r + 1 < ND && s_pre[r + 1] <= t) r++;
        const u64 at = (u64)s_g[r] + (t - s_pre[r]);
        s_val[cidx[at]] = val[at];
    }
    __syncthreads();
    for (u32 t = tid; t < len; t += PA_T) { const u32 v = s_val[t]; up_store<OUT>(out, lo + t, v); mysum += v; }
    if (OUT == UP_U32 && total) { const u64 b = block_sum<u64, PA_T>(mysum, s_sum); if (tid == 0 && b) atomicAdd(total, (unsigned long long)b); }
}

template <int OUT, int TILE>
__global__ __launch_bounds__(512) void k_unpermute_paged(const u64 *__restrict__ pool, const uint2 *__restrict__ vtab, PageTab pt, u32 nreg, u32 rowbits,
                                                         u64 n, void *__restrict__ out, unsigned long long *total)
{
    constexpr int T = 512, ND = 256;
    __shared__ u32 s_val[TILE];
    __shared__ u32 s_pre[ND + 1], s_v[ND], s_pg0[ND];
    __shared__ u32 scan_lds[T / IVX_WAVE + 1];
    __shared__ u64 s_sum[T / IVX_WAVE];
    const u32 tid = threadIdx.x;
    const u64 t0 = (u64)blockIdx.x * TILE;
    const u32 len = (u32)(t0 + TILE < n ? (u64)TILE : n - t0);
    const u32 rowmask = rowbits >= 32 ? 0xFFFFFFFFu : (1u << rowbits) - 1u;
    const u32 pmask = (1u << pt.lgpg) - 1u;
    u32 v = 0, c = 0;
    if (tid < nreg) { const uint2 vc = vtab[(u64)blockIdx.x * ND + tid]; v = vc.x; c = vc.y; }
    u32 tot;
    const u32 ex = block_excl_scan<u32, T>(c, scan_lds, &tot);
    if (tid < ND) { s_pre[tid] = ex; s_v[tid] = v; s_pg0[tid] = c ? pt.ptab[(u64)tid * pt.pstride + (v >> pt.lgpg)] - 1u : 0u; }
    if (tid == 0) s_pre[ND] = tot;
// ... 137 lines not shown
{
    if (*unsorted == 0) return;
    const u32 r = blockIdx.x * WR_T + threadIdx.x;
    if (r > nreg) return;
    if (r == nreg) { rfirst[r] = offs1[nh1 - 1]; return; }
    const u32 sp = r / G, sub = r - sp * G;
    const u32 nt = tprefix[sp + 1] - tprefix[sp];
    rfirst[r] = nt ? hist2[(u64)G * tprefix[sp] + (u64)sub * nt] : offs1[(u64)sp * nblk1];
}

__global__ __launch_bounds__(WR_T) void k_sorted_bounds(JoinIndexView ix, const u32 *__restrict__ pkey, const i32 *__restrict__ ps, u64 n,
                                                        u32 nreg, u32 *__restrict__ rfirst, const u32 *unsorted)
{
    __shared__ i32 s_origin[KT_MAX];
    __shared__ u32 s_last[KT_MAX], s_kreg[KT_MAX];
    if (*unsorted != 0) return;
    KeyTab kt;
    keytab_load(ix, s_origin, s_last, s_kreg, kt);
    __syncthreads();
    const u32 r = blockIdx.x * WR_T + threadIdx.x;
    if (r > nreg) return;
    u64 lo = 0, hi = n;
    auto body = [&](auto klds_tag) {
        constexpr bool KLDS = decltype(klds_tag)::value;
        while (lo < hi) { const u64 mid = lo + ((hi - lo) >> 1); if (region_of<KLDS>(ix, kt, s_origin, s_last, s_kreg, pkey ? pkey[mid] : 0u, ps[mid]) < r) lo = mid + 1; else hi = mid; }
    };
    KEYTAB_DISPATCH(kt, body);
    rfirst[r] = (u32)lo;
}

}

static inline bool cols_aligned16(const u32 *key, const i32 *s, const i32 *e) { return (((uintptr_t)key | (uintptr_t)s | (uintptr_t)e) & 15) == 0; }
static constexpr u64 IN_COLS = (1ull << WS_IN_START) | (1ull << WS_IN_END);

ivx_status ivx_route_flat(ivx_ctx *ctx, const JoinIndexView &jv, const u32 *key, const i32 *s, const i32 *e, u64 n, u32 adj,
                          u32 ndig, bool ids16, u32 max_tiles, ivx_routed *R)
{
    hipStream_t st = ctx->stream;
    const u32 chunk = part_chunk(n, max_tiles);
    const u32 nblk = (u32)((n + chunk - 1) / chunk);
    const u64 nh = (u64)ndig * nblk + 1;
    u32 *hist; u64 *pse; void *ids;
    IVX_TRY(ctx->get_scratch(WS_SORTHIST, nh * sizeof(u32), (void **)&hist));
    IVX_TRY(ctx->get_scratch(WS_T0, n * sizeof(u64), (void **)&pse));
    IVX_TRY(ctx->get_scratch(WS_T1, n * (ids16 ? sizeof(unsigned short) : sizeof(u32)), &ids));
    u32 *unsorted = (u32 *)(ctx->d_scalars + 10);
    IVX_HIP(ctx, hipMemsetAsync(hist + (nh - 1), 0, sizeof(u32), st));
    IVX_HIP(ctx, hipMemsetAsync(unsorted, 0, sizeof(u32), st));
    ivx_status scan = IVX_OK;
    with_bools([&](auto vec, auto wide, auto i16) {
        constexpr int ND = IVX_B(wide) ? 1024 : 256;
        using RowT = typename std::conditional<IVX_B(i16), unsigned short, u32>::type;
        hipLaunchKernelGGL((k_part_hist<IVX_B(vec), ND>), dim3(nblk), dim3(PA_T), 0, st, jv, key, s, n, nblk, chunk, hist, adj, unsorted);
        if ((scan = ivx_scan_exclusive_u32(ctx, hist, nh)) != IVX_OK) return;
        hipLaunchKernelGGL((k_part_scatter<IVX_B(vec), RowT, ND>), dim3(nblk), dim3(PA_T), 0, st, jv, key, s, e, n, nblk, (const u32 *)hist, pse, (RowT *)ids, chunk, adj, (const u32 *)unsorted);
    }, cols_aligned16(key, s, e), ndig > 256, ids16);
    IVX_TRY(scan);
    IVX_HIP(ctx, hipGetLastError());
    *R = ivx_routed{};
    R->form = IVX_ROWS_FLAT; R->se = pse; R->rfirst = hist; R->nblk = nblk; R->chunk = chunk; R->ndig = ndig; R->unsorted = unsorted;
    if (ids16) R->cidx = (const unsigned short *)ids; else R->ids = (const u32 *)ids;
    R->ds = s; R->de = e; R->adj = adj;
    R->slots = (1ull << WS_SORTHIST) | (1ull << WS_T0) | (1ull << WS_T1) | IN_COLS;
    return IVX_OK;
}

ivx_status ivx_route_paged(ivx_ctx *ctx, const JoinIndexView &jv, u32 nreg, const u32 *key, const i32 *s, const i32 *e, u64 n,
                           const ivx_paged_opts &o, ivx_routed *R)
{
    hipStream_t st = ctx->stream;
    const bool wide = nreg > IVX_MAXREG;
    const bool half = o.packed && !wide;
    const u32 tile = wide ? PA_T * 8u : half ? 512u * 16u : PA_T * 12u;
    u32 rowbits = 1;
    while (rowbits < 32 && (n - 1) >> rowbits) rowbits++;
    if (o.filter) rowbits = 32;
    u32 lgpg = 14;
    while (lgpg < 31 && (n >> lgpg) > 4096) lgpg++;
    const u64 pstride = (n >> lgpg) + 2;
    const u64 npages = (n >> lgpg) + nreg + 1;
    const u64 ntiles = (n + tile - 1) / tile;
    ivx_route_ctl *ctl; u32 *ptab; u64 *pool; u32 *prow = nullptr; uint2 *vtab = nullptr; void *rest = nullptr;
    *R = ivx_routed{};
    R->slots = (1ull << WS_SORTHIST) | (1ull << WS_T0) | (1ull << WS_T1) | (1ull << WS_T2) | IN_COLS;
    IVX_TRY(ctx->get_scratch(WS_SORTHIST, sizeof(ivx_route_ctl), (void **)&ctl));
    IVX_TRY(ctx->get_scratch(WS_T2, (size_t)nreg * pstride * sizeof(u32), (void **)&ptab));
    IVX_TRY(ctx->get_scratch(WS_T0, (size_t)(npages << lgpg) * sizeof(u64), (void **)&pool));
    if (o.rowval) IVX_TRY(ctx->get_scratch(WS_T1, (size_t)ntiles * 256 * sizeof(uint2), (void **)&vtab));
    else if (!o.packed) IVX_TRY(ctx->get_scratch(WS_T1, (size_t)(npages << lgpg) * sizeof(u32), (void **)&prow));
    else if (o.lean) IVX_TRY(ctx->get_scratch(WS_T1, (size_t)fp_max_batches(n, nreg) * sizeof(FpRest) + (size_t)(n + 64) * sizeof(u64), &rest));
    if (rest) { R->rest = (FpRest *)rest; R->rest_rows = (u64 *)(R->rest + fp_max_batches(n, nreg)); }
    if (o.rowval && o.lean) { IVX_TRY(ctx->get_scratch(WS_T3, (size_t)(n + 64) * sizeof(u64), (void **)&R->rest_rows)); R->slots |= 1ull << WS_T3; }
    {
        const u32 nctl = (u32)(offsetof(ivx_route_ctl, rfirst) / sizeof(u32));
        const u64 nptab = (u64)nreg * pstride;
        u64 cg = (nptab / 4 + 256 * 8 - 1) / (256 * 8);
        cg = cg < (nctl + 255) / 256 ? (nctl + 255) / 256 : (cg > 1024 ? 1024 : cg);
        hipLaunchKernelGGL(k_route_clear, dim3((u32)cg), dim3(256), 0, st, (u32 *)ctl, nctl, ptab, nptab, o.zero2);
    }
    const PageTab pt{ptab, (u32)pstride, lgpg};
    const u32 tiles = n >= (16u << 20) ? 4u : n >= (4u << 20) ? 2u : 1u;
    const u32 chunk1 = tile * tiles;
    const u32 nblk1 = (u32)((n + chunk1 - 1) / chunk1);
    with_bools([&](auto vec, auto klds, auto filt, auto pk) {
        auto part = [&](auto kern, u32 threads) {
            hipLaunchKernelGGL(kern, dim3(nblk1), dim3(threads), 0, st, jv, key, s, e, n, chunk1, ctl->rcur, pt, &ctl->pool_next, pool, prow, rowbits, o.adj, vtab);
        };
        if (half) part(k_part_onepass<IVX_B(vec), 256, 16, IVX_B(klds), IVX_B(filt), true, 512>, 512u);
        else if (wide) part(k_part_onepass<IVX_B(vec), 1024, 8, IVX_B(klds), IVX_B(filt), IVX_B(pk)>, (u32)PA_T);
        else part(k_part_onepass<IVX_B(vec), 256, 12, IVX_B(klds), IVX_B(filt), IVX_B(pk)>, (u32)PA_T);
    }, cols_aligned16(key, s, e), jv.nkeys <= KT_MAX, o.filter, o.packed);
    if (o.rowval && !o.lean) hipLaunchKernelGGL(k_page_bounds, dim3(1), dim3(1024), 0, st, (const u32 *)ctl->rcur, nreg, ctl->rfirst);
    else hipLaunchKernelGGL(k_chunk_bounds, dim3(1), dim3(1024), 0, st, (const u32 *)ctl->rcur, nreg, ctl->rfirst, ctl->cfirst);
    IVX_HIP(ctx, hipGetLastError());
    R->form = IVX_ROWS_PAGED; R->se = pool; R->ids = prow; R->rfirst = ctl->rfirst; R->pt = pt; R->packed = o.packed; R->rowbits = rowbits;
    R->all_routed = !o.filter; R->ctl = ctl; R->vtab = vtab; R->ds = s; R->de = e; R->adj = o.adj;
    return IVX_OK;
}

ivx_status ivx_route_two_level(ivx_ctx *ctx, const JoinIndexView &jv, u32 nreg, const u32 *key, const i32 *s, const i32 *e, u64 n, ivx_routed *R)
{
    hipStream_t st = ctx->stream;
    u32 *unsorted = (u32 *)(ctx->d_scalars + 10);
    const u32 G = (nreg + IVX_MAXREG_WIDE - 1) / IVX_MAXREG_WIDE;
    if (G > P2_SUBMAX) return ctx->fail(IVX_ERR_INVALID, "overlap index with too many probe regions");
    const u32 nsuper = (nreg + G - 1) / G;
    const uint2 split = make_uint2(G, (u32)(((1ull << 32) + G - 1) / G));
    const u32 chunk = part_chunk(n);
    const u32 nblk1 = (u32)((n + chunk - 1) / chunk);
    const u64 nh1 = (u64)1024 * nblk1 + 1;
    const u32 grid2 = (u32)(n / PA_TILE) + nsuper + 1;
    const u64 nh2 = (u64)G * grid2 + 1;
    u32 *hist1, *hist2, *tprefix, *prow1, *rfirst, *prow2; u64 *pse1, *pse2; unsigned char *sub1;
    IVX_TRY(ctx->get_scratch(WS_SORTHIST, nh1 * sizeof(u32), (void **)&hist1));
    IVX_TRY(ctx->get_scratch(WS_T0, n * sizeof(u64), (void **)&pse1));
    IVX_TRY(ctx->get_scratch(WS_T1, n * sizeof(u32), (void **)&prow1));
    IVX_TRY(ctx->get_scratch(WS_T2, n, (void **)&sub1));
    IVX_TRY(ctx->get_scratch(WS_SA0, n * sizeof(u64), (void **)&pse2));
    IVX_TRY(ctx->get_scratch(WS_SA1, n * sizeof(u32), (void **)&prow2));
    IVX_TRY(ctx->get_scratch(WS_T4, ((size_t)nsuper + 1) * sizeof(u32), (void **)&tprefix));
    IVX_TRY(ctx->get_scratch(WS_T5, nh2 * sizeof(u32), (void **)&hist2));
    IVX_TRY(ctx->get_scratch(WS_T6, ((size_t)nreg + 1) * sizeof(u32), (void **)&rfirst));
    IVX_HIP(ctx, hipMemsetAsync(hist1 + (nh1 - 1), 0, sizeof(u32), st));
    IVX_HIP(ctx, hipMemsetAsync(hist2, 0, nh2 * sizeof(u32), st));
    IVX_HIP(ctx, hipMemsetAsync(unsorted, 0, sizeof(u32), st));
    ivx_status scan = IVX_OK;
    with_bools([&](auto vec) {
        hipLaunchKernelGGL((k_part_hist<IVX_B(vec), 1024, true>), dim3(nblk1), dim3(PA_T), 0, st, jv, key, s, n, nblk1, chunk, hist1, 0u, unsorted, split);
        if ((scan = ivx_scan_exclusive_u32(ctx, hist1, nh1)) != IVX_OK) return;
        hipLaunchKernelGGL((k_part_scatter<IVX_B(vec), u32, 1024, true>), dim3(nblk1), dim3(PA_T), 0, st, jv, key, s, e, n, nblk1, (const u32 *)hist1, pse1, prow1, chunk, 0u, (const u32 *)unsorted, split, sub1);
    }, cols_aligned16(key, s, e));
    IVX_TRY(scan);
    hipLaunchKernelGGL(k_p2_layout, dim3(1), dim3(1024), 0, st, (const u32 *)hist1, nblk1, nsuper, tprefix, (const u32 *)unsorted);
    hipLaunchKernelGGL(k_p2_hist, dim3(grid2), dim3(PA_T), 0, st, (const unsigned char *)sub1, (const u32 *)hist1, nblk1, nsuper, (const u32 *)tprefix, G, hist2, (const u32 *)unsorted);
    IVX_TRY(ivx_scan_exclusive_u32(ctx, hist2, nh2));
    hipLaunchKernelGGL(k_p2_scatter, dim3(grid2), dim3(PA_T), 0, st, (const unsigned char *)sub1, (const u64 *)pse1, (const u32 *)prow1, (const u32 *)hist1, nblk1, nsuper,
                       (const u32 *)tprefix, G, (const u32 *)hist2, pse2, prow2, (const u32 *)unsorted);
    const u32 bgrid = (nreg + 1 + WR_T - 1) / WR_T;
    hipLaunchKernelGGL(k_p2_bounds, dim3(bgrid), dim3(WR_T), 0, st, nreg, G, nsuper, (const u32 *)hist1, nblk1, nh1, (const u32 *)tprefix, (const u32 *)hist2, rfirst, (const u32 *)unsorted);
    hipLaunchKernelGGL(k_sorted_bounds, dim3(bgrid), dim3(WR_T), 0, st, jv, key, s, n, nreg, rfirst, (const u32 *)unsorted);
    IVX_HIP(ctx, hipGetLastError());
    *R = ivx_routed{};
    R->form = IVX_ROWS_TABLE; R->se = pse2; R->ids = prow2; R->rfirst = rfirst; R->unsorted = unsorted; R->ds = s; R->de = e;
    R->slots = IN_COLS;
    for (int slot : {WS_SORTHIST, WS_T0, WS_T1, WS_T2, WS_SA0, WS_SA1, WS_T4, WS_T5, WS_T6}) R->slots |= 1ull << slot;
    return IVX_OK;
}

ivx_status ivx_unroute_values(ivx_ctx *ctx, const ivx_routed &R, u32 nreg, int kind, const u32 *val, u64 n, void *out, u64 *d_total, int sorted_done)
{
    hipStream_t st = ctx->stream;
    auto go = [&](auto out_tag) {
        constexpr int O = decltype(out_tag)::value;
        if (R.form == IVX_ROWS_PAGED) {
            constexpr u32 TILE = 512u * 16u;
            hipLaunchKernelGGL((k_unpermute_paged<O, (int)TILE>), dim3((u32)((n + TILE - 1) / TILE)), dim3(512), 0, st, R.se, R.vtab, R.pt, nreg, R.rowbits, n, out, (unsigned long long *)d_total);
        } else with_bools([&](auto wide) {
            constexpr int ND = IVX_B(wide) ? 1024 : 256;
            hipLaunchKernelGGL((k_unpermute<O, ND>), dim3(R.nblk), dim3(PA_T), 0, st, val, R.cidx, R.rfirst, R.nblk, R.chunk, (u32)ND, n, out, R.unsorted, (unsigned long long *)d_total, sorted_done);
        }, R.ndig > 256);
    };
    switch (kind) {
    case IVX_RV_COVERAGE: go(std::integral_constant<int, UP_I64S>{}); break;
    case IVX_RV_COUNT: go(std::integral_constant<int, UP_I64>{}); break;
    case IVX_RV_PER_ROW: go(std::integral_constant<int, UP_U32>{}); break;
    default: go(std::integral_constant<int, UP_U8>{}); break;
    }
    IVX_HIP(ctx, hipGetLastError());
    return IVX_OK;
}

ivx_status ivx_route_rows(ivx_ctx *ctx, const JoinIndexView &rv, const u32 *key, const i32 *s, const i32 *e, u64 n, u32 adj, ivx_routed *out)
{
    return ivx_route_flat(ctx, rv, key, s, e, n, adj, 1024, true, 1, out);
}

// ... 14 lines not shown
```

Before: 35.26 billion overlap-pairs/s.

## Trim launches on the routed fill path: fuse bounds scan, skip clears, defer slow fallback

Folds the per-region bounds scan into the last workgroup of the partition kernel and moves the scalar zeroing there, so two small kernel launches go away. The route-table clear is skipped when the previous fill left the control block and page table clean. The slow-path fallback probe is no longer launched speculatively: the fast kernel flags slow mode, and the host reruns only when asked. The build also defers the filter kernel onto the overlapped tail and skips the index-ready wait on the same stream. The k_fill_rest kernel is reworked to wave-cooperative cell scans. This adds cross-call state that can go stale, a last-block atomic pattern, and a possible host round trip when the slow path is taken.

```diff
diff --git a/datafusion-bio-functions_amd/csrc/ivx_capi.hip b/datafusion-bio-functions_amd/csrc/ivx_capi.hip
--- a/datafusion-bio-functions_amd/csrc/ivx_capi.hip
+++ b/datafusion-bio-functions_amd/csrc/ivx_capi.hip
@@ -23,8 +23,10 @@
     ivx_buf &b = scratch[slot];
     if (sub_plan.valid && ((sub_plan.slots >> slot) & 1)) sub_plan.valid = false;
     if (join_plan.valid && ((join_plan.rows.slots >> slot) & 1)) join_plan.valid = false;
+    if (slot == WS_SORTHIST || slot == WS_T2) route_clean = false;
     if (bytes < 256) bytes = 256;
     if (b.cap < bytes) {
+        if (slot == WS_SORTHIST || slot == WS_T2) route_ctl = route_ptab = nullptr;
         size_t want = bytes + bytes / 8;
         if (mem_limit) {
             const u64 others = reserved() - b.cap;
@@ -316,6 +318,7 @@
     IVX_HIP(c, hipStreamSynchronize(c->stream));
     if (c->aux) { IVX_HIP(c, hipStreamSynchronize(c->aux)); c->tail_pending = false; }
     c->sub_plan.valid = false; c->join_plan.valid = false;
+    c->route_clean = false; c->route_ctl = c->route_ptab = nullptr;
     while (c->scratch_bytes > keep_bytes) {
         int big = -1;
         for (int i = 0; i < IVX_NSCRATCH; i++)
@@ -462,7 +465,7 @@
     ivx_join_plan &pl = ctx->join_plan;
     const bool planned = regions && mode == JP_FILL && pl.valid && !getenv("IVX_NO_PLAN") && pl.mem == mem && memcmp(pl.in, in, sizeof(in)) == 0 && pl.n == n &&
                          pl.ix == (const void *)ix && pl.ix_serial == ix->serial && pl.stream == ctx->stream;
-    if (ix->ready != nullptr && !(regions && !planned)) IVX_HIP(ctx, hipStreamWaitEvent(ctx->stream, ix->ready, 0));
+    if (ix->ready != nullptr && !(regions && !planned && ctx->stream == ix->built_on)) IVX_HIP(ctx, hipStreamWaitEvent(ctx->stream, ix->ready, 0));
     if (!planned) {
         IVX_TRY(stage_in(ctx, mem, WS_IN_KEY, key, n, &dk));
         IVX_TRY(stage_in(ctx, mem, WS_IN_START, start, n, &ds));
@@ -475,16 +478,21 @@
     IVX_TRY(stage_out(ctx, mem, WS_OUT_D, pidx, cap, &d_p));
     const bool defer_clear = regions && !planned;
     if (!defer_clear) IVX_HIP(ctx, hipMemsetAsync(ctx->d_scalars, 0, 2 * sizeof(u64), ctx->stream));
-    {
-        KernelTimer t(ctx);
-        if (regions) {
-            if (!planned) pl.valid = false;
-            const ivx_status st = ivx_join_probe_regions(ctx, ix->jv, ix->jv_nreg, mode, dk, ds, de, n, d_b, d_p, cap, ctx->d_scalars, planned, ix->jv_filter, ix->jv_pk24,
-                                                         ix->jv_fast_unknown ? 2 : (ix->jv_fast ? 1 : 0), planned ? nullptr : ix->ready, defer_clear);
-            if (st != IVX_OK) { pl.valid = false; return st; }
-            if (mode == JP_COUNT && pl.valid) { memcpy(pl.in, in, sizeof(in)); pl.mem = mem; pl.n = n; pl.ix = ix; pl.ix_serial = ix->serial; pl.stream = ctx->stream; }
-        }
-        else if (rowval) IVX_TRY(ivx_rowval_probe_regions(ctx, ix->jv, ix->jv_nreg, mode == JP_PER_ROW ? IVX_RV_PER_ROW : IVX_RV_EXISTS, dk, ds, de, n, 0,
+    ctx->fill_told = 0;
+    auto probe_regions = [&]() -> ivx_status {
+        KernelTimer t(ctx);
+        if (!planned) pl.valid = false;
+        ctx->fill_told = 0;
+        const ivx_status st = ivx_join_probe_regions(ctx, ix->jv, ix->jv_nreg, mode, dk, ds, de, n, d_b, d_p, cap, ctx->d_scalars, planned, ix->jv_filter, ix->jv_pk24,
+                                                     ix->jv_fast_unknown ? 2 : (ix->jv_fast ? 1 : 0), planned ? nullptr : ix->ready, defer_clear);
+        if (st != IVX_OK) { pl.valid = false; return st; }
+        if (mode == JP_COUNT && pl.valid) { memcpy(pl.in, in, sizeof(in)); pl.mem = mem; pl.n = n; pl.ix = ix; pl.ix_serial = ix->serial; pl.stream = ctx->stream; }
+        return IVX_OK;
+    };
+    if (regions) IVX_TRY(probe_regions());
+    else {
+        KernelTimer t(ctx);
+        if (rowval) IVX_TRY(ivx_rowval_probe_regions(ctx, ix->jv, ix->jv_nreg, mode == JP_PER_ROW ? IVX_RV_PER_ROW : IVX_RV_EXISTS, dk, ds, de, n, 0,
                                                           mode == JP_PER_ROW ? (void *)d_row : (void *)d_ex, ctx->d_scalars, ix->jv_filter, ix->jv_pk24, ix->jv_fast && !ix->jv_fast_unknown));
         else if (n && (mode == JP_PER_ROW || mode == JP_EXISTS) && ix->nroute_nreg > 0 && rowval_routed_ok(n))
             IVX_TRY(ivx_join_rowval_routed(ctx, ix, mode, dk, ds, de, n, d_row, d_ex, ctx->d_scalars));
@@ -494,8 +502,20 @@
     if (mode != JP_EXISTS) {
         IVX_HIP(ctx, hipMemcpyAsync(ctx->h_scalars, ctx->d_scalars, 2 * sizeof(u64), hipMemcpyDeviceToHost, ctx->stream));
         IVX_HIP(ctx, hipStreamSynchronize(ctx->stream));
+        if (ctx->fill_told & ivx_ctx::FILL_ASKS_SLOW) {
+            const bool slow = (ctx->h_scalars[1] & IVX_FW_SLOW) != 0;
+            ix->jv_fast = !slow; ix->jv_fast_unknown = false;
+            if (slow) {
+                if (!defer_clear) IVX_HIP(ctx, hipMemsetAsync(ctx->d_scalars, 0, 2 * sizeof(u64), ctx->stream));
+                IVX_TRY(probe_regions());
+                IVX_HIP(ctx, hipMemcpyAsync(ctx->h_scalars, ctx->d_scalars, 2 * sizeof(u64), hipMemcpyDeviceToHost, ctx->stream));
+                IVX_HIP(ctx, hipStreamSynchronize(ctx->stream));
+            }
+        }
         tot = ctx->h_scalars[0];
-        if (ctx->h_scalars[1]) { ctx->join_plan.valid = false; return ctx->fail(IVX_ERR_HIP, "internal error: the probe met an unpublished page of routed rows"); }
+        if (ctx->fill_told & ivx_ctx::FILL_CLEANS) ctx->route_clean = tot <= cap && ctx->h_scalars[1] == 0;
+        ctx->fill_told = 0;
+        if (ctx->h_scalars[1] & IVX_FW_MISS) { ctx->join_plan.valid = false; return ctx->fail(IVX_ERR_HIP, "internal error: the probe met an unpublished page of routed rows"); }
     }
     if (mode == JP_COUNT && regions && pl.valid) pl.total = tot;
     if (total) *total = tot;
diff --git a/datafusion-bio-functions_amd/csrc/ivx_internal.hpp b/datafusion-bio-functions_amd/csrc/ivx_internal.hpp
--- a/datafusion-bio-functions_amd/csrc/ivx_internal.hpp
+++ b/datafusion-bio-functions_amd/csrc/ivx_internal.hpp
@@ -38,11 +38,13 @@
 struct PageTab { u32 *ptab; u32 pstride, lgpg; };
 struct ivx_route_ctl {
     u32 rcur[1024];
-    u32 pool_next, pad0[3];
+    u32 pool_next;
+    u32 done, pad0[2];
     u32 rest_n[2], pad1[2];
     u32 rfirst[1032];
     u32 cfirst[1032];
 };
+enum { IVX_FW_MISS = 1u , IVX_FW_SLOW = 2u  };
 struct FpRest;
 enum {
     IVX_ROWS_FLAT = 0,
@@ -95,6 +97,11 @@
     ivx_join_plan join_plan;
     ivx_metrics metrics{};
     u64 mem_limit = 0;
+    bool route_clean = false;
+    const void *route_ctl = nullptr, *route_ptab = nullptr;
+    u64 route_nptab = 0;
+    enum { FILL_CLEANS = 1, FILL_ASKS_SLOW = 2 };
+    int fill_told = 0;
     u64 fill_hint = 0;
     u64 scratch_bytes = 0, building_bytes = 0;
     hipStream_t aux = nullptr;
@@ -224,8 +231,9 @@
     u32 jv_nreg = 0;
     bool jv_filter = false;
     bool jv_pk24 = false;
-    bool jv_fast = false;
-    bool jv_fast_unknown = false;
+    mutable bool jv_fast = false;
+    mutable bool jv_fast_unknown = false;
+    hipStream_t built_on = nullptr;
     hipEvent_t ready = nullptr;
     RankGridView gs{}, ge{};
     CoverageView cv{};
diff --git a/datafusion-bio-functions_amd/csrc/ivx_join.hip b/datafusion-bio-functions_amd/csrc/ivx_join.hip
--- a/datafusion-bio-functions_amd/csrc/ivx_join.hip
+++ b/datafusion-bio-functions_amd/csrc/ivx_join.hip
@@ -648,10 +648,14 @@
     if (filter_mode) { zr.big = (uint4 *)fbits; zr.nbig = (u32)(fwords / 4); }
     IVX_TRY(ivx_keystats_len(ctx, key, s, n, nkeys, kmin, kmax, kcnt, errflag, 1u, e, lenhist, &zr));
     const u32 grid = ivx_stream_grid(n, BT * 2, 16384);
-    hipLaunchKernelGGL(k_join_layout, dim3(1), dim3(1024), 0, st, kmin, kmax, kcnt, nkeys, n, origin, span, lbase, hdr, maxcells, kreg, rkey, (const u32 *)lenhist, (u32)(regcap - 1), fbase, filter_mode, lb_try ? 1 : 0, (const u32 *)errflag);
-    if (filter_mode) hipLaunchKernelGGL(k_join_filter, dim3(grid), dim3(BT), 0, st, key, s, e, n, nkeys, (const i32 *)origin, (const u32 *)span, (const u32 *)fbase, (const u32 *)hdr, fbits);
     const bool want_route = ix->kind == IVX_KIND_OVERLAP && n >= (4u << 20);
     overlap = overlap && ctx->overlap && ctx->aux != nullptr && !want_route && n >= (1u << 16);
+    hipLaunchKernelGGL(k_join_layout, dim3(1), dim3(1024), 0, st, kmin, kmax, kcnt, nkeys, n, origin, span, lbase, hdr, maxcells, kreg, rkey, (const u32 *)lenhist, (u32)(regcap - 1), fbase, filter_mode, lb_try ? 1 : 0, (const u32 *)errflag);
+    auto launch_filter = [&]() {
+        hipLaunchKernelGGL(k_join_filter, dim3(grid), dim3(BT), 0, st, key, s, e, n, nkeys, (const i32 *)origin, (const u32 *)span, (const u32 *)fbase, (const u32 *)hdr, fbits);
+    };
+    if (filter_mode && !overlap) launch_filter();
+    bool late_filter = false;
     hipStream_t tail_st = st;
     struct TailGuard {
         ivx_ctx *c; bool armed = false;
@@ -669,6 +673,11 @@
         q_lds = lb_try && ((const u32 *)(ctx->h_scalars + 32))[HDR_LBUILD] != 0;
         q_global = !q_lds;
         guard.armed = true;
+        late_filter = filter_mode && ((const u32 *)(ctx->h_scalars + 32))[HDR_FG] != 0xFFFFFFFFu;
+        if (late_filter) {
+            launch_filter();
+            IVX_HIP(ctx, hipEventRecord(ctx->ev_fork, st));
+        }
     }
     if (q_lds)
         hipLaunchKernelGGL(k_lbuild_tiles, dim3(lb_tiles), dim3(LB_T), 0, tail_st, key, s, e, n, nkeys, (const i32 *)origin, (const u32 *)kreg, hdr,
@@ -693,6 +702,7 @@
     IVX_HIP(ctx, hipGetLastError());
     if (overlap) {
         if (ix->ready == nullptr) IVX_HIP(ctx, hipEventCreateWithFlags(&ix->ready, hipEventDisableTiming));
+        if (late_filter) IVX_HIP(ctx, hipStreamWaitEvent(ctx->aux, ctx->ev_fork, 0));
         IVX_HIP(ctx, hipEventRecord(ix->ready, ctx->aux));
         IVX_HIP(ctx, hipEventRecord(ctx->tail_ev, ctx->aux));
         ctx->tail_pending = true;
@@ -716,6 +726,7 @@
     ix->jv.binstart = binstart; ix->jv.ent = ent; ix->jv.hdr = hdr; ix->jv.nkeys = nkeys;
     ix->jv.kreg = kreg; ix->jv.rkey = rkey; ix->jv.rdesc = rdesc;
     ix->jv.fbits = fbits; ix->jv.fbase = fbase;
+    ix->built_on = st;
     return IVX_OK;
 }
 
diff --git a/datafusion-bio-functions_amd/csrc/ivx_join.hpp b/datafusion-bio-functions_amd/csrc/ivx_join.hpp
--- a/datafusion-bio-functions_amd/csrc/ivx_join.hpp
+++ b/datafusion-bio-functions_amd/csrc/ivx_join.hpp
@@ -18,7 +18,7 @@
 }
 
 template <class F>
-__device__ __forceinline__ void walk_ent(const JoinIndexView &ix, u32 sh0, u32 lev0, u32 nlev, u32 k, i32 qs, i32 qe, F &&f)
+__device__ __forceinline__ void walk_cells(const JoinIndexView &ix, u32 sh0, u32 lev0, u32 nlev, u32 k, i32 qs, i32 qe, F &&f)
 {
     if (k >= ix.nkeys) return;
     if (ix.kcnt[k] == 0) return;
@@ -41,12 +41,18 @@
             if (blo > bhi) continue;
         }
         const u32 base = ix.lbase[(u64)l * ix.nkeys + k];
-        const u32 a = ix.binstart[base + blo], b = ix.binstart[base + bhi + 1];
+        f(ix.binstart[base + blo], ix.binstart[base + bhi + 1]);
+    }
+}
+template <class F>
+__device__ __forceinline__ void walk_ent(const JoinIndexView &ix, u32 sh0, u32 lev0, u32 nlev, u32 k, i32 qs, i32 qe, F &&f)
+{
+    walk_cells(ix, sh0, lev0, nlev, k, qs, qe, [&](u32 a, u32 b) {
         for (u32 j = a; j < b; j++) {
             const ivx_ent x = ix.ent[j];
             if (x.s <= qe && x.e >= qs) f(x);
         }
-    }
+    });
 }
 template <class F>
 __device__ __forceinline__ void walk(const JoinIndexView &ix, u32 sh0, u32 lev0, u32 nlev, u32 k, i32 qs, i32 qe, F &&f)
diff --git a/datafusion-bio-functions_amd/csrc/ivx_regions_probe.hip b/datafusion-bio-functions_amd/csrc/ivx_regions_probe.hip
--- a/datafusion-bio-functions_amd/csrc/ivx_regions_probe.hip
+++ b/datafusion-bio-functions_amd/csrc/ivx_regions_probe.hip
@@ -327,10 +327,9 @@
                                                         unsigned long long *cursor, u32 prow_stride, u32 adj,
                                                         const u32 *unsorted, PageTab pt = PageTab{nullptr, 0u, 0u},
                                                         const u32 *bsel = nullptr, const i32 *__restrict__ ps_in = nullptr, const i32 *__restrict__ pe_in = nullptr,
-                                                        u32 rowbits = 32, const u32 *only_if_set = nullptr)
+                                                        u32 rowbits = 32)
 {
     constexpr bool FILL = MODE == 1;
-    if (only_if_set != nullptr && *only_if_set == 0u) return;
     const u32 rowmask = rowbits >= 32 ? 0xFFFFFFFFu : (1u << rowbits) - 1u;
     const u32 maxlen = pk_maxlen(rowbits);
     static_assert(!PK || PAGED, "packed rows come from the one-pass partition");
@@ -622,13 +621,16 @@
                                                     u32 drain)
 {
     if (bsel != nullptr && *bsel != (u32)B) return;
-    if (ix.hdr[HDR_SLOW] != 0u) return;
+    if (ix.hdr[HDR_SLOW] != 0u) {
+        if (blockIdx.x == 0 && threadIdx.x == 0) atomicOr((unsigned int *)(cursor + 1), (unsigned int)IVX_FW_SLOW);
+        return;
+    }
     IVX_PROBE_LDS(true)
     __shared__ u32 s_cfirst[IVX_MAXREG_WIDE + 2];
     __shared__ u32 s_wat[RP_NSLOT][RP_W];
     __shared__ u32 s_stash[DRAIN ? RP_W : 1][RP_STASH];
     const u32 wv = __builtin_amdgcn_readfirstlane(threadIdx.x / IVX_WAVE), ln = lane_id();
-    auto miss = [&]() { if (ln == 0) atomicOr((unsigned int *)(cursor + 1), 1u); };
+    auto miss = [&]() { if (ln == 0) atomicOr((unsigned int *)(cursor + 1), (unsigned int)IVX_FW_MISS); };
     LeanRows<B, const u64> rows;
     if (!rows.init(ix, s_cfirst, cfirst, rcur, pt, pool, rowbits)) return;
     Slice S;
@@ -741,43 +743,115 @@
 }
 
 __global__ __launch_bounds__(256) void k_fill_rest(JoinIndexView ix, const u64 *__restrict__ pool, PageTab pt, const FpRest *__restrict__ rest,
-                                                   const u64 *__restrict__ rest_rows, const u32 *__restrict__ rest_n, u32 *__restrict__ ob,
+                                                   const u64 *__restrict__ rest_rows, ivx_route_ctl *ctl, u32 *__restrict__ ob,
                                                    u32 *__restrict__ op, u64 cap, unsigned long long *cursor, const i32 *__restrict__ ps_in,
                                                    const i32 *__restrict__ pe_in, u32 rowbits)
 {
-    const u32 nbat = rest_n[0], nrow = rest_n[1];
-    if (nbat == 0 && nrow == 0) return;
+    __shared__ u32 s_rows[IVX_MAXREG_WIDE + 1];
+    __shared__ u32 s_last, s_fits;
+    const u32 nbat = ctl->rest_n[0], nrow = ctl->rest_n[1];
     const u32 wpb = blockDim.x / IVX_WAVE, ln = lane_id();
-    const u32 sh0 = ix.hdr[HDR_SH0], nlev = ix.hdr[HDR_NLEV];
-    auto rows64 = [&](bool ok, u32 r, u32 v) {
-        i32 qs = 0, qe = -1; u32 row = 0, k = 0;
-        if (ok) {
-            const auto e = rest_row(ix, pt, pool, r, v, rowbits, ps_in, pe_in, 0u, [&]() { atomicOr((unsigned int *)(cursor + 1), 1u); });
-            qs = e.qs; qe = e.qe; row = e.row;
-            k = ix.rkey[r];
-        }
-        u32 m = 0;
-        if (ok) walk(ix, sh0, 0, nlev, k, qs, qe, [&](u32) { m++; });
-        const u32 inc = wave_incl_scan(m);
-        const u32 tot = __shfl(inc, IVX_WAVE - 1, IVX_WAVE);
-        if (tot == 0) return;
-        unsigned long long g = 0;
-        if (ln == 0) g = atomicAdd(cursor, (unsigned long long)tot);
-        g = __shfl(g, 0, IVX_WAVE);
-        if (g + tot > cap) return;
-        u64 at = g + inc - m;
-        if (m) walk(ix, sh0, 0, nlev, k, qs, qe, [&](u32 brow) { ob[at] = brow; op[at] = row; at++; });
-    };
     const u32 wave = blockIdx.x * wpb + threadIdx.x / IVX_WAVE, nwave = gridDim.x * wpb;
-    for (u32 i0 = wave * IVX_WAVE; i0 < nrow; i0 += nwave * IVX_WAVE) {
-        const bool ok = i0 + ln < nrow;
-        const u64 e = ok ? rest_rows[i0 + ln] : 0ull;
-        rows64(ok, (u32)(e >> 32), (u32)e);
-    }
-    for (u32 b = wave; b < nbat; b += nwave) {
-        const FpRest w = rest[b];
-        for (u32 t0 = 0; t0 < w.cnt; t0 += IVX_WAVE) rows64(t0 + ln < w.cnt, w.r, w.first + t0 + ln);
-    }
+    if (nbat != 0 || nrow != 0) {
+        const u32 sh0 = ix.hdr[HDR_SH0], nlev = ix.hdr[HDR_NLEV];
+        auto miss = [&]() { atomicOr((unsigned int *)(cursor + 1), (unsigned int)IVX_FW_MISS); };
+        auto row1 = [&](u32 r, u32 v) {
+            const auto e = rest_row(ix, pt, pool, r, v, rowbits, ps_in, pe_in, 0u, miss);
+            const i32 qs = e.qs, qe = e.qe;
+            const u32 k = ix.rkey[r];
+            auto trip = [&](u32 j0, u32 b, u32 &brow) {
+                const u32 j = j0 + ln;
+                if (j >= b) return false;
+                const ivx_ent x = ix.ent[j];
+                brow = x.row;
+                return x.s <= qe && x.e >= qs;
+            };
+            u32 tot = 0, trips = 0, brow0 = 0;
+            u64 mm0 = 0;
+            walk_cells(ix, sh0, 0, nlev, k, qs, qe, [&](u32 a, u32 b) {
+                for (u32 j0 = a; j0 < b; j0 += IVX_WAVE) {
+                    u32 brow = 0;
+                    const u64 mm = __ballot(trip(j0, b, brow));
+                    if (trips == 0) { brow0 = brow; mm0 = mm; }
+                    trips++;
+                    tot += (u32)__popcll(mm);
+                }
+            });
+            if (tot == 0) return;
+            unsigned long long g = 0;
+            if (ln == 0) g = atomicAdd(cursor, (unsigned long long)tot);
+            g = __shfl(g, 0, IVX_WAVE);
+            if (g + tot > cap) return;
+            auto put = [&](u64 mm, u32 brow) {
+                if ((mm >> ln) & 1ull) { const u64 at = g + mask_rank(mm); ob[at] = brow; op[at] = e.row; }
+                g += (u32)__popcll(mm);
+            };
+            if (trips == 1) { put(mm0, brow0); return; }
+            walk_cells(ix, sh0, 0, nlev, k, qs, qe, [&](u32 a, u32 b) {
+                for (u32 j0 = a; j0 < b; j0 += IVX_WAVE) {
+                    u32 brow = 0;
+                    const u64 mm = __ballot(trip(j0, b, brow));
+                    put(mm, brow);
+                }
+            });
+        };
+        auto rows64 = [&](bool ok, u32 r, u32 v) {
+            i32 qs = 0, qe = -1; u32 row = 0, k = 0;
+            if (ok) {
+                const auto e = rest_row(ix, pt, pool, r, v, rowbits, ps_in, pe_in, 0u, miss);
+                qs = e.qs; qe = e.qe; row = e.row;
+                k = ix.rkey[r];
+            }
+            u32 m = 0;
+            if (ok) walk(ix, sh0, 0, nlev, k, qs, qe, [&](u32) { m++; });
+            const u32 inc = wave_incl_scan(m);
+            const u32 tot = __shfl(inc, IVX_WAVE - 1, IVX_WAVE);
+            if (tot == 0) return;
+            unsigned long long g = 0;
+            if (ln == 0) g = atomicAdd(cursor, (unsigned long long)tot);
+            g = __shfl(g, 0, IVX_WAVE);
+            if (g + tot > cap) return;
+            u64 at = g + inc - m;
+            if (m) walk(ix, sh0, 0, nlev, k, qs, qe, [&](u32 brow) { ob[at] = brow; op[at] = row; at++; });
+        };
+#ifdef IVX_REST_BY_WAVE
+        if (wave < nrow) {
+            const u64 e = rest_rows[wave];
+            row1((u32)__builtin_amdgcn_readfirstlane((u32)(e >> 32)), (u32)__builtin_amdgcn_readfirstlane((u32)e));
+        }
+        const u32 done1 = nwave;
+#else
+        const u32 done1 = 0;
+#endif
+        for (u32 i0 = done1 + wave * IVX_WAVE; i0 < nrow; i0 += nwave * IVX_WAVE) {
+            const bool ok = i0 + ln < nrow;
+            const u64 e = ok ? rest_rows[i0 + ln] : 0ull;
+            rows64(ok, (u32)(e >> 32), (u32)e);
+        }
+        for (u32 b = wave; b < nbat; b += nwave) {
+            const FpRest w = rest[b];
+            for (u32 t0 = 0; t0 < w.cnt; t0 += IVX_WAVE) rows64(t0 + ln < w.cnt, w.r, w.first + t0 + ln);
+        }
+    }
+    __syncthreads();
+    if (threadIdx.x == 0) s_last = __hip_atomic_fetch_add(&ctl->done, 1u, __ATOMIC_RELAXED, __HIP_MEMORY_SCOPE_AGENT) == gridDim.x - 1u ? 1u : 0u;
+    __syncthreads();
+    if (s_last == 0u) return;
+    if (threadIdx.x == 0) {
+        const unsigned long long pairs = atomicAdd(cursor, 0ull);
+        const unsigned int fault = atomicOr((unsigned int *)(cursor + 1), 0u);
+        s_fits = pairs <= cap && fault == 0u ? 1u : 0u;
+    }
+    const u32 nreg = ix.hdr[HDR_NREG];
+    for (u32 r = threadIdx.x; r < nreg; r += blockDim.x) s_rows[r] = ctl->rcur[r];
+    __syncthreads();
+    if (s_fits == 0u) { if (threadIdx.x == 0) ctl->done = 0; return; }
+    for (u32 r = threadIdx.x / IVX_WAVE; r < nreg; r += wpb) {
+        const u32 rows = s_rows[r];
+        const u32 np = rows ? ((rows - 1u) >> pt.lgpg) + 1u : 0u;
+        for (u32 p = ln; p < np; p += IVX_WAVE) pt.ptab[(u64)r * pt.pstride + p] = 0u;
+    }
+    for (u32 i = threadIdx.x; i < (u32)(offsetof(ivx_route_ctl, rfirst) / sizeof(u32)); i += blockDim.x) ((u32 *)ctl)[i] = 0u;
 }
 
 #ifndef IVX_RV_WPS
@@ -1143,13 +1217,13 @@
 
 template <int MODE, int B>
 void launch_probe_regions(hipStream_t st, const JoinIndexView &jv, const ivx_routed &R, u32 grid, u32 *ob, u32 *op, u64 cap,
-                          unsigned long long *cur, const u32 *bsel = nullptr, const u32 *only_if_set = nullptr)
+                          unsigned long long *cur, const u32 *bsel = nullptr)
 {
     const u32 vpb = RP_VGRID / grid;
     if (R.form == IVX_ROWS_PAGED) {
         auto go = [&](auto pk) {
             hipLaunchKernelGGL((k_probe_regions<MODE, B, false, true, IVX_B(pk)>), dim3(grid), dim3(RP_T), 0, st, jv, (const void *)R.se, (const void *)R.ids, R.rfirst, 1u, vpb,
-                               ob, op, cap, cur, 1u, R.adj, (const u32 *)nullptr, R.pt, bsel, R.ds, R.de, R.rowbits, only_if_set);
+                               ob, op, cap, cur, 1u, R.adj, (const u32 *)nullptr, R.pt, bsel, R.ds, R.de, R.rowbits);
         };
         if constexpr (MODE >= RV_COUNT) go(std::true_type{}); else with_bools(go, R.packed);
         return;
@@ -1203,7 +1277,6 @@
         if (bsel) { f(int_tag<8>{}); f(int_tag<4>{}); f(int_tag<2>{}); f(int_tag<1>{}); }
         else with_rows_per_lane(fill_rows_per_lane(K, hint, n), f);
     };
-    const u32 *slow_gate = nullptr;
     if (lean_rows_ok(R) && fast != 0 && !K.lean_off && R.rest != nullptr) {
         u32 *rest_n = R.ctl->rest_n;
         if (reused) IVX_HIP(ctx, hipMemsetAsync(rest_n, 0, 2 * sizeof(u32), st));
@@ -1214,12 +1287,12 @@
                                    (const u32 *)bsel, R.rowbits, R.rest, R.rest_rows, rest_n, drain);
             }, drain != 0);
         });
-        hipLaunchKernelGGL(k_fill_rest, dim3(512), dim3(256), 0, st, jv, R.se, R.pt, (const FpRest *)R.rest, (const u64 *)R.rest_rows, (const u32 *)rest_n, ob, op, cap, cur, R.ds, R.de, R.rowbits);
+        hipLaunchKernelGGL(k_fill_rest, dim3(512), dim3(256), 0, st, jv, R.se, R.pt, (const FpRest *)R.rest, (const u64 *)R.rest_rows, R.ctl, ob, op, cap, cur, R.ds, R.de, R.rowbits);
         IVX_HIP(ctx, hipGetLastError());
-        if (fast == 1) return IVX_OK;
-        slow_gate = jv.hdr + HDR_SLOW;
-    }
-    every_b([&](auto b) { launch_probe_regions<1, decltype(b)::value>(st, jv, R, RP_GRID, ob, op, cap, cur, bsel, slow_gate); });
+        ctx->fill_told = ivx_ctx::FILL_CLEANS | (fast == 2 ? ivx_ctx::FILL_ASKS_SLOW : 0);
+        return IVX_OK;
+    }
+    every_b([&](auto b) { launch_probe_regions<1, decltype(b)::value>(st, jv, R, RP_GRID, ob, op, cap, cur, bsel); });
     IVX_HIP(ctx, hipGetLastError());
     return IVX_OK;
 }
diff --git a/datafusion-bio-functions_amd/csrc/ivx_regions_route.hip b/datafusion-bio-functions_amd/csrc/ivx_regions_route.hip
--- a/datafusion-bio-functions_amd/csrc/ivx_regions_route.hip
+++ b/datafusion-bio-functions_amd/csrc/ivx_regions_route.hip
@@ -336,9 +336,9 @@
 
 template <bool VEC, int ND, int I, bool KLDS, bool FILT, bool PK, int T = PA_T>
 __global__ __launch_bounds__(T, 4) void k_part_onepass(JoinIndexView ix, const u32 *__restrict__ pkey, const i32 *__restrict__ ps,
-                                                       const i32 *__restrict__ pe, u64 n, u32 chunk, u32 *__restrict__ rcur, PageTab pt,
-                                                       u32 *pool_next, u64 *__restrict__ out_se, u32 *__restrict__ out_row, u32 rowbits,
-                                                       u32 adj = 0, uint2 *__restrict__ vtab = nullptr)
+                                                       const i32 *__restrict__ pe, u64 n, u32 chunk, ivx_route_ctl *ctl, PageTab pt,
+                                                       u64 *__restrict__ out_se, u32 *__restrict__ out_row, u32 rowbits,
+                                                       u32 adj = 0, uint2 *__restrict__ vtab = nullptr, u64 *zero2 = nullptr)
 {
     constexpr int TILE = T * I;
     static_assert(ND <= T, "one thread per region");
@@ -351,8 +351,10 @@
     __shared__ u32 scan_lds[T / IVX_WAVE + 1];
     __shared__ i32 s_origin[KT_MAX];
     __shared__ u32 s_span[KT_MAX], s_kreg[KT_MAX], s_fbase[KT_MAX];
+    __shared__ u32 s_last;
 
     const u32 tid = threadIdx.x;
+    u32 *const rcur = ctl->rcur, *const pool_next = &ctl->pool_next;
     KeyTab2 kt;
     keytab2_load<KLDS>(ix, s_origin, s_span, s_kreg, s_fbase, kt, FILT);
     const u32 pmask = (1u << pt.lgpg) - 1u;
@@ -475,38 +477,36 @@
         }
         __syncthreads();
     }
-}
-
-__global__ __launch_bounds__(1024) void k_page_bounds(const u32 *__restrict__ rcur, u32 nreg, u32 *__restrict__ rfirst)
-{
-    __shared__ u32 red[1024 / IVX_WAVE + 1];
-    const u32 t = threadIdx.x;
-    u32 tot;
-    const u32 ex = block_excl_scan<u32, 1024>(t < nreg ? rcur[t] : 0u, red, &tot);
-    if (t < nreg) rfirst[t] = ex;
-    if (t == 0) rfirst[nreg] = tot;
-}
-
-__global__ __launch_bounds__(1024) void k_chunk_bounds(const u32 *__restrict__ rcur, u32 nreg, u32 *__restrict__ rfirst, u32 *__restrict__ cfirst)
-{
-    __shared__ u32 red[1024 / IVX_WAVE + 1];
-    const u32 t = threadIdx.x;
-    const u32 rows = t < nreg ? rcur[t] : 0u;
-    u32 tot;
-    const u32 ex = block_excl_scan<u32, 1024>(rows, red, &tot);
-    if (t < nreg) rfirst[t] = ex;
-    if (t == 0) rfirst[nreg] = tot;
-    __syncthreads();
-    const u32 ec = block_excl_scan<u32, 1024>((rows + FP_CHUNK - 1) / FP_CHUNK, red, &tot);
-    if (t < nreg) cfirst[t] = ec;
-    if (t == 0) cfirst[nreg] = tot;
-}
-
-__global__ __launch_bounds__(256) void k_route_clear(u32 *__restrict__ ctl, u32 nctl, u32 *__restrict__ ptab, u64 nptab, u64 *zero2)
+    if (blockIdx.x == 0 && tid == 0 && zero2 != nullptr) { zero2[0] = 0; zero2[1] = 0; }
+    if (tid == 0) s_last = __hip_atomic_fetch_add(&ctl->done, 1u, __ATOMIC_RELAXED, __HIP_MEMORY_SCOPE_AGENT) == gridDim.x - 1u ? 1u : 0u;
+    __syncthreads();
+    if (s_last == 0u) return;
+    const u32 nreg = ix.hdr[HDR_NREG];
+    constexpr int PER = 1024 / T;
+    static_assert(PER * T == 1024, "the region tables are scanned by one workgroup, 1024 / T counters a thread");
+    u32 rows[PER], rsum = 0, csum = 0;
+#pragma unroll
+    for (int k = 0; k < PER; k++) {
+        const u32 r = tid * PER + k;
+        rows[k] = r < nreg ? atomicOr(&rcur[r], 0u) : 0u;
+        rsum += rows[k]; csum += (rows[k] + FP_CHUNK - 1) / FP_CHUNK;
+    }
+    u32 rtot, ctot;
+    u32 rex = block_excl_scan<u32, T>(rsum, scan_lds, &rtot);
+    u32 cex = block_excl_scan<u32, T>(csum, scan_lds, &ctot);
+#pragma unroll
+    for (int k = 0; k < PER; k++) {
+        const u32 r = tid * PER + k;
+        if (r < nreg) { ctl->rfirst[r] = rex; ctl->cfirst[r] = cex; }
+        rex += rows[k]; cex += (rows[k] + FP_CHUNK - 1) / FP_CHUNK;
+    }
+    if (tid == 0) { ctl->rfirst[nreg] = rtot; ctl->cfirst[nreg] = ctot; ctl->done = 0; }
+}
+
+__global__ __launch_bounds__(256) void k_route_clear(u32 *__restrict__ ctl, u32 nctl, u32 *__restrict__ ptab, u64 nptab)
 {
     const u64 i = (u64)blockIdx.x * 256 + threadIdx.x, step = (u64)gridDim.x * 256;
     if (i < nctl) ctl[i] = 0;
-    if (i < 2 && zero2) zero2[i] = 0;
     uint4 *p4 = (uint4 *)ptab;
     for (u64 j = i; j < nptab / 4; j += step) p4[j] = make_uint4(0u, 0u, 0u, 0u);
     if (i < (nptab & 3)) ptab[(nptab & ~3ull) + i] = 0;
@@ -810,6 +810,7 @@
     const u64 npages = (n >> lgpg) + nreg + 1;
     const u64 ntiles = (n + tile - 1) / tile;
     ivx_route_ctl *ctl; u32 *ptab; u64 *pool; u32 *prow = nullptr; uint2 *vtab = nullptr; void *rest = nullptr;
+    const bool was_clean = ctx->route_clean;
     *R = ivx_routed{};
     R->slots = (1ull << WS_SORTHIST) | (1ull << WS_T0) | (1ull << WS_T1) | (1ull << WS_T2) | IN_COLS;
     IVX_TRY(ctx->get_scratch(WS_SORTHIST, sizeof(ivx_route_ctl), (void **)&ctl));
@@ -820,27 +821,27 @@
     else if (o.lean) IVX_TRY(ctx->get_scratch(WS_T1, (size_t)fp_max_batches(n, nreg) * sizeof(FpRest) + (size_t)(n + 64) * sizeof(u64), &rest));
     if (rest) { R->rest = (FpRest *)rest; R->rest_rows = (u64 *)(R->rest + fp_max_batches(n, nreg)); }
     if (o.rowval && o.lean) { IVX_TRY(ctx->get_scratch(WS_T3, (size_t)(n + 64) * sizeof(u64), (void **)&R->rest_rows)); R->slots |= 1ull << WS_T3; }
-    {
+    const u64 nptab = (u64)nreg * pstride;
+    if (!(was_clean && ctx->route_ctl == (const void *)ctl && ctx->route_ptab == (const void *)ptab && nptab <= ctx->route_nptab)) {
         const u32 nctl = (u32)(offsetof(ivx_route_ctl, rfirst) / sizeof(u32));
-        const u64 nptab = (u64)nreg * pstride;
         u64 cg = (nptab / 4 + 256 * 8 - 1) / (256 * 8);
         cg = cg < (nctl + 255) / 256 ? (nctl + 255) / 256 : (cg > 1024 ? 1024 : cg);
-        hipLaunchKernelGGL(k_route_clear, dim3((u32)cg), dim3(256), 0, st, (u32 *)ctl, nctl, ptab, nptab, o.zero2);
-    }
+        hipLaunchKernelGGL(k_route_clear, dim3((u32)cg), dim3(256), 0, st, (u32 *)ctl, nctl, ptab, nptab);
+        ctx->route_nptab = nptab;
+    }
+    ctx->route_ctl = ctl; ctx->route_ptab = ptab;
     const PageTab pt{ptab, (u32)pstride, lgpg};
     const u32 tiles = n >= (16u << 20) ? 4u : n >= (4u << 20) ? 2u : 1u;
     const u32 chunk1 = tile * tiles;
     const u32 nblk1 = (u32)((n + chunk1 - 1) / chunk1);
     with_bools([&](auto vec, auto klds, auto filt, auto pk) {
         auto part = [&](auto kern, u32 threads) {
-            hipLaunchKernelGGL(kern, dim3(nblk1), dim3(threads), 0, st, jv, key, s, e, n, chunk1, ctl->rcur, pt, &ctl->pool_next, pool, prow, rowbits, o.adj, vtab);
+            hipLaunchKernelGGL(kern, dim3(nblk1), dim3(threads), 0, st, jv, key, s, e, n, chunk1, ctl, pt, pool, prow, rowbits, o.adj, vtab, o.zero2);
         };
         if (half) part(k_part_onepass<IVX_B(vec), 256, 16, IVX_B(klds), IVX_B(filt), true, 512>, 512u);
         else if (wide) part(k_part_onepass<IVX_B(vec), 1024, 8, IVX_B(klds), IVX_B(filt), IVX_B(pk)>, (u32)PA_T);
         else part(k_part_onepass<IVX_B(vec), 256, 12, IVX_B(klds), IVX_B(filt), IVX_B(pk)>, (u32)PA_T);
     }, cols_aligned16(key, s, e), jv.nkeys <= KT_MAX, o.filter, o.packed);
-    if (o.rowval && !o.lean) hipLaunchKernelGGL(k_page_bounds, dim3(1), dim3(1024), 0, st, (const u32 *)ctl->rcur, nreg, ctl->rfirst);
-    else hipLaunchKernelGGL(k_chunk_bounds, dim3(1), dim3(1024), 0, st, (const u32 *)ctl->rcur, nreg, ctl->rfirst, ctl->cfirst);
     IVX_HIP(ctx, hipGetLastError());
     R->form = IVX_ROWS_PAGED; R->se = pool; R->ids = prow; R->rfirst = ctl->rfirst; R->pt = pt; R->packed = o.packed; R->rowbits = rowbits;
     R->all_routed = !o.filter; R->ctl = ctl; R->vtab = vtab; R->ds = s; R->de = e; R->adj = o.adj;
```

Result: slower. 34.69 billion overlap-pairs/s (-1.6%).
